# QZ1-boy/FCVSR

Hardware: AMD Instinct MI355X
Metric: SR frames/sec (7-frame window, 4x 180x320->720x1280) + PSNR vs ref (higher is better)
Workload: dtype bf16

## Files before the change

### fcvsr_amd/csrc/conv_mfma.hip

```cpp
#include <stdlib.h>
#include "common.h"
#include "mfma_util.h"
#include "conv_res.h"

namespace fcvsr {

constexpr int kTW = 32, kCK = 64, kLD = kCK + 8;

struct MGroup {
  View src[3];
  View res[2];
  View dst;
  float* gc_partial;
  int B, H, W;
  int tiles_x, tiles_y;
  int tile_begin;
};

struct MfmaArgs {
  int n_groups;
  MGroup g[3];
  int n_src, n_res;
  int seg_c[3];
  int cin_total, cin16, cin_pad, cout, cout_pad, n_nblk;
  const uint16_t* w;
  const float* bias;
  int act;
  float slope;
  const float* slope_ptr;
  float rs[2];
  int ps;
  int flat;
  int src16, dst16;
  int dstbf;
  int res16;
  int gc16;
  const float* gc_wmask;
  int planar;
  int sub2;
  int dbg;
};

struct EpiCtx {
  int act, n_res, ps, flat, H, W, b, dst16, dstbf, sub2, cq4;
  float slope, rs0, rs1;
  long long npix;
  View res0, res1, dst;
};

template <bool BF16>
__device__ __forceinline__ bool epilogue_quad(const EpiCtx& e, float4 v, const float* bias, int cout, int n, int py, int px,
                                              long long pflat, float4* xo) {
  bool pok = e.flat ? (pflat < e.npix) : ((py < e.H) && (px < e.W));
  if (e.sub2) {
    pok = pok && !((py | px) & 1);
    py >>= 1;
    px >>= 1;
  }
  if (!pok || n >= cout) return false;
  const bool full = (n + 3 < cout);
  float x[4] = {v.x, v.y, v.z, v.w};
  if (bias) {
    if (full) {
      const float4 b4 = *reinterpret_cast<const float4*>(bias + n);
      x[0] += b4.x; x[1] += b4.y; x[2] += b4.z; x[3] += b4.w;
    } else {
#pragma unroll
      for (int q = 0; q < 4; ++q) if (n + q < cout) x[q] += bias[n + q];
    }
  }
#pragma unroll
  for (int q = 0; q < 4; ++q) {
    x[q] = x[q] >= 0.f ? x[q] : x[q] * e.slope;
  }
  const int sp_r = e.ps ? n / e.cq4 : 0;
  const int c_r = e.ps ? n - sp_r * e.cq4 : n;
#pragma unroll
  for (int ri = 0; ri < 2; ++ri) {
    if (ri < e.n_res) {
      const View& rv = ri == 0 ? e.res0 : e.res1;
      const float rs = ri == 0 ? e.rs0 : e.rs1;
      const int o = (e.flat ? (int)pflat * (int)rv.sx : (e.b * (int)rv.sb + py * (int)rv.sy + px * (int)rv.sx));
      if (full && rv.sc == 1 && !e.ps) {
        const float4 r4 = *reinterpret_cast<const float4*>(rv.p + o + n);
        x[0] = fmaf(rs, r4.x, x[0]); x[1] = fmaf(rs, r4.y, x[1]); x[2] = fmaf(rs, r4.z, x[2]); x[3] = fmaf(rs, r4.w, x[3]);
      } else {
#pragma unroll
        for (int q = 0; q < 4; ++q) {
          const int ch = e.ps ? 4 * (c_r + q) + sp_r : n + q;
          if (n + q < cout) x[q] = fmaf(rs, rv.p[o + ch * (int)rv.sc], x[q]);
        }
      }
    }
  }
  const View& d = e.dst;
  int o;
  int nn = n;
  if (e.ps) {
    int qy = py, qx = px, qb = e.b;
    if (e.flat) {
      qx = (int)(pflat % e.W);
      qy = (int)((pflat / e.W) % e.H);
      qb = (int)(pflat / ((long long)e.W * e.H));
    }
    const int sp = n / e.cq4;
    nn = n - sp * e.cq4;
    o = qb * (int)d.sb + (2 * qy + (sp >> 1)) * (int)d.sy + (2 * qx + (sp & 1)) * (int)d.sx;
  } else {
    o = (e.flat ? (int)pflat * (int)d.sx : (e.b * (int)d.sb + py * (int)d.sy + px * (int)d.sx));
  }
  if (e.dst16) {
    uint16_t* dp = reinterpret_cast<uint16_t*>(d.p);
    const uint2 pk = e.dstbf ? cvt4<true>(make_float4(x[0], x[1], x[2], x[3])) : cvt4<false>(make_float4(x[0], x[1], x[2], x[3]));
    if (full && d.sc == 1) {
      *reinterpret_cast<uint2*>(dp + o + nn) = pk;
    } else {
      const uint16_t hv[4] = {(uint16_t)(pk.x & 0xffff), (uint16_t)(pk.x >> 16), (uint16_t)(pk.y & 0xffff), (uint16_t)(pk.y >> 16)};
#pragma unroll
      for (int q = 0; q < 4; ++q) if (n + q < cout) dp[o + (nn + q) * (int)d.sc] = hv[q];
    }
  } else if (full && d.sc == 1) {
    *reinterpret_cast<float4*>(d.p + o + nn) = make_float4(x[0], x[1], x[2], x[3]);
  } else {
#pragma unroll
    for (int q = 0; q < 4; ++q) if (n + q < cout) d.p[o + (nn + q) * (int)d.sc] = x[q];
  }
  *xo = make_float4(x[0], n + 1 < cout ? x[1] : 0.f, n + 2 < cout ? x[2] : 0.f, n + 3 < cout ? x[3] : 0.f);
  return true;
}

template <bool BF16>
__device__ __forceinline__ void epilogue_oct(const EpiCtx& e, float4 va, float4 vb, const float* bias, int n, int py, int px,
                                             long long pflat) {
  bool pok = e.flat ? (pflat < e.npix) : ((py < e.H) && (px < e.W));
  if (e.sub2) {
    pok = pok && !((py | px) & 1);
    py >>= 1;
    px >>= 1;
  }
  if (!pok) return;
  float x[8] = {va.x, va.y, va.z, va.w, vb.x, vb.y, vb.z, vb.w};
  if (bias) {
    const float4 b0 = *reinterpret_cast<const float4*>(bias + n), b1 = *reinterpret_cast<const float4*>(bias + n + 4);
    x[0] += b0.x; x[1] += b0.y; x[2] += b0.z; x[3] += b0.w; x[4] += b1.x; x[5] += b1.y; x[6] += b1.z; x[7] += b1.w;
  }
#pragma unroll
  for (int q = 0; q < 8; ++q) {
    x[q] = x[q] >= 0.f ? x[q] : x[q] * e.slope;
  }
#pragma unroll
  for (int ri = 0; ri < 2; ++ri) {
    if (ri < e.n_res) {
      const View& rv = ri == 0 ? e.res0 : e.res1;
      const float rs = ri == 0 ? e.rs0 : e.rs1;
      const int o = (e.flat ? (int)pflat * (int)rv.sx : (e.b * (int)rv.sb + py * (int)rv.sy + px * (int)rv.sx));
      if (rv.sc == 1) {
        const float4 r0 = *reinterpret_cast<const float4*>(rv.p + o + n), r1 = *reinterpret_cast<const float4*>(rv.p + o + n + 4);
        x[0] = fmaf(rs, r0.x, x[0]); x[1] = fmaf(rs, r0.y, x[1]); x[2] = fmaf(rs, r0.z, x[2]); x[3] = fmaf(rs, r0.w, x[3]);
        x[4] = fmaf(rs, r1.x, x[4]); x[5] = fmaf(rs, r1.y, x[5]); x[6] = fmaf(rs, r1.z, x[6]); x[7] = fmaf(rs, r1.w, x[7]);
      } else {
#pragma unroll
        for (int q = 0; q < 8; ++q) x[q] = fmaf(rs, rv.p[o + (n + q) * (int)rv.sc], x[q]);
      }
    }
  }
  const View& d = e.dst;
  const int o = (e.flat ? (int)pflat * (int)d.sx : (e.b * (int)d.sb + py * (int)d.sy + px * (int)d.sx));
  uint2 lo, hi;
  if (e.dstbf) { lo = cvt4<true>(make_float4(x[0], x[1], x[2], x[3])); hi = cvt4<true>(make_float4(x[4], x[5], x[6], x[7])); }
  else { lo = cvt4<false>(make_float4(x[0], x[1], x[2], x[3])); hi = cvt4<false>(make_float4(x[4], x[5], x[6], x[7])); }
  *reinterpret_cast<uint4*>(reinterpret_cast<uint16_t*>(d.p) + o + n) = make_uint4(lo.x, lo.y, hi.x, hi.y);
}

__device__ __forceinline__ long long uniform64(long long v) {
  const unsigned lo = __builtin_amdgcn_readfirstlane((unsigned)v), hi = __builtin_amdgcn_readfirstlane((unsigned)((unsigned long long)v >> 32));
  return (long long)(((unsigned long long)hi << 32) | lo);
}
__device__ __forceinline__ long long sel3(int i, long long a, long long b, long long c) { return i == 0 ? a : (i == 1 ? b : c); }
typedef unsigned __attribute__((ext_vector_type(4))) cm_u32x4_t;
typedef float __attribute__((ext_vector_type(4))) cm_f32x4_t;
typedef __attribute__((address_space(1))) cm_u32x4_t cm_guint4_t;
typedef __attribute__((address_space(1))) cm_f32x4_t cm_gfloat4_t;
__device__ __forceinline__ uint4 gld_u4(long long addr) { const cm_u32x4_t v = *reinterpret_cast<const cm_guint4_t*>((unsigned long long)addr); return make_uint4(v.x, v.y, v.z, v.w); }
__device__ __forceinline__ float4 gld_f4(long long addr) { const cm_f32x4_t v = *reinterpret_cast<const cm_gfloat4_t*>((unsigned long long)addr); return make_float4(v.x, v.y, v.z, v.w); }

template <bool BF16, int NT, int KS, int MW, bool WD>
__global__ __launch_bounds__(256, MW == 1 ? (WD ? (NT == 128 ? 2 : 3) : (NT == 128 ? 3 : 4)) : 2) void conv_mfma_kernel(MfmaArgs a) {
  constexpr bool FLAT = KS == 1;
  constexpr int kTH = 4 * MW;
  constexpr int PAD = KS / 2;
  constexpr int HH = kTH + 2 * PAD, HWD = kTW + 2 * PAD;
  constexpr int NF = NT / 32;
  constexpr int WLOADS = NT * kCK * 2 / 16 / 256;
  extern __shared__ __align__(16) uint16_t lds[];
  uint16_t* A_s = lds;
  uint16_t* B_s = lds + HH * HWD * kLD;

  const int tid = threadIdx.x;
  const int lane = tid & 63, wave = tid >> 6;
  const int r = lane & 31, h = lane >> 5;

  int wid = blockIdx.x;
  {
    const int nwg = gridDim.x, q = nwg >> 3, rr = nwg & 7, xcd = wid & 7, loc = wid >> 3;
    wid = (xcd < rr ? xcd * (q + 1) : rr * (q + 1) + (xcd - rr) * q) + loc;
  }
  const int nb = wid % a.n_nblk;
  const int tflat = wid / a.n_nblk;
  int gi = 0;
  if (a.n_groups > 1 && tflat >= a.g[1].tile_begin) gi = 1;
  if (a.n_groups > 2 && tflat >= a.g[2].tile_begin) gi = 2;
  const MGroup& G = a.g[gi];
  const int tl = tflat - G.tile_begin;
  const int n0 = nb * NT;
  int b, ty0, tx0;
  long long flat0 = 0;
  const long long npix = (long long)G.B * G.H * G.W;
  if (a.flat) {
    flat0 = (long long)tl * (kTH * kTW);
    b = 0; ty0 = 0; tx0 = 0;
  } else {
    const int per_img = G.tiles_x * G.tiles_y;
    b = tl / per_img;
    const int t2 = tl % per_img;
    ty0 = (t2 / G.tiles_x) * kTH;
    tx0 = (t2 % G.tiles_x) * kTW;
  }

  f32x16_t acc[MW][NF];
#pragma unroll
  for (int m = 0; m < MW; ++m)
#pragma unroll
    for (int nf = 0; nf < NF; ++nf)
#pragma unroll
      for (int i = 0; i < 16; ++i) acc[m][nf][i] = 0.f;

  for (int c0 = 0; c0 < a.cin16; c0 += kCK) {
    const int ck = (a.cin16 - c0) < kCK ? (a.cin16 - c0) : kCK;
    __syncthreads();
    if (a.planar) {
      constexpr int NHP = HH * HWD;
      const View sv = G.src[0];
      const int cpad = a.cin16;
      for (int idx = tid; idx < NHP * cpad; idx += 256) {
        const int hp = idx % NHP, c = idx / NHP;
        const int hy = hp / HWD, hx = hp - hy * HWD;
        const int iy = ty0 + hy - PAD, ix = tx0 + hx - PAD;
        float v = 0.f;
        if (c < a.cin_total && iy >= 0 && iy < G.H && ix >= 0 && ix < G.W && !(a.dbg & 1))
          v = sv.p[(long long)b * sv.sb + (long long)iy * sv.sy + (long long)ix * sv.sx + (long long)c * sv.sc];
        const uint2 pk = cvt4<BF16>(make_float4(v, 0.f, 0.f, 0.f));
        A_s[hp * kLD + c] = (uint16_t)(pk.x & 0xffff);
      }
    } else if (!a.src16) {
      constexpr int NHP = HH * HWD;
      constexpr int ITERS = (NHP * 16 + 255) / 256;
      const int q = tid & 15;
      const int c = c0 + q * 4;
      const bool cok = (c < a.cin_total) && !(a.dbg & 1);
      int s_ = 0, cl = c;
      if (cl >= a.seg_c[0]) { cl -= a.seg_c[0]; s_ = 1; if (cl >= a.seg_c[1]) { cl -= a.seg_c[1]; s_ = 2; } }
      const int si = cok ? s_ : 0;
      const long long sp0 = sel3(si, uniform64((long long)G.src[0].p), uniform64((long long)G.src[1].p), uniform64((long long)G.src[2].p));
      const long long ssb = sel3(si, uniform64(G.src[0].sb), uniform64(G.src[1].sb), uniform64(G.src[2].sb));
      const long long ssy = sel3(si, uniform64(G.src[0].sy), uniform64(G.src[1].sy), uniform64(G.src[2].sy));
      const long long ssx = sel3(si, uniform64(G.src[0].sx), uniform64(G.src[1].sx), uniform64(G.src[2].sx));
      const long long sbase = sp0 + 4 * ((FLAT ? 0ll : (long long)b * ssb) + (cok ? cl : 0));
      constexpr int UNR = 8;
#pragma unroll 1
      for (int it0 = 0; it0 < ITERS; it0 += UNR) {
        float4 v[UNR];
        bool ok[UNR];
#pragma unroll
        for (int u = 0; u < UNR; ++u) {
          const int hp = (tid >> 4) + (it0 + u) * 16;
          long long off;
          if (FLAT) {
            const long long p = flat0 + hp;
            ok[u] = cok && hp < NHP && p < npix;
            off = (p < npix ? p : npix - 1) * ssx;
          } else {
            const int hy = hp / HWD, hx = hp - hy * HWD;
            const int iy = ty0 + hy - PAD, ix = tx0 + hx - PAD;
            ok[u] = cok && hp < NHP && iy >= 0 && iy < G.H && ix >= 0 && ix < G.W;
            const int cy = iy < 0 ? 0 : (iy > G.H - 1 ? G.H - 1 : iy), cx = ix < 0 ? 0 : (ix > G.W - 1 ? G.W - 1 : ix);
            off = (long long)cy * ssy + (long long)cx * ssx;
          }
          v[u] = gld_f4(sbase + 4 * off);
        }
#pragma unroll
        for (int u = 0; u < UNR; ++u)
          if (!ok[u]) v[u] = make_float4(0.f, 0.f, 0.f, 0.f);
#pragma unroll
        for (int u = 0; u < UNR; ++u) {
          const int hp = (tid >> 4) + (it0 + u) * 16;
          if (hp < NHP) *reinterpret_cast<uint2*>(A_s + hp * kLD + q * 4) = cvt4<BF16>(v[u]);
        }
      }
    } else {
      constexpr int NHP = HH * HWD;
      constexpr int ITERS = (NHP * 8 + 255) / 256;
      const int q = tid & 7;
      const int c = c0 + q * 8;
      const bool cok = (c < a.cin_total) && !(a.dbg & 1);
      int s_ = 0, cl = c;
      if (cl >= a.seg_c[0]) { cl -= a.seg_c[0]; s_ = 1; if (cl >= a.seg_c[1]) { cl -= a.seg_c[1]; s_ = 2; } }
      const int si = cok ? s_ : 0;
      const long long sp0 = sel3(si, uniform64((long long)G.src[0].p), uniform64((long long)G.src[1].p), uniform64((long long)G.src[2].p));
      const long long ssb = sel3(si, uniform64(G.src[0].sb), uniform64(G.src[1].sb), uniform64(G.src[2].sb));
      const long long ssy = sel3(si, uniform64(G.src[0].sy), uniform64(G.src[1].sy), uniform64(G.src[2].sy));
      const long long ssx = sel3(si, uniform64(G.src[0].sx), uniform64(G.src[1].sx), uniform64(G.src[2].sx));
      const long long sbase = sp0 + 2 * ((FLAT ? 0ll : (long long)b * ssb) + (cok ? cl : 0));
      constexpr int UNR = 8;
#pragma unroll 1
      for (int it0 = 0; it0 < ITERS; it0 += UNR) {
        uint4 v[UNR];
        bool ok[UNR];
#pragma unroll
        for (int u = 0; u < UNR; ++u) {
          const int hp = (tid >> 3) + (it0 + u) * 32;
          long long off;
          if (FLAT) {
            const long long p = flat0 + hp;
            ok[u] = cok && hp < NHP && p < npix;
            off = (p < npix ? p : npix - 1) * ssx;
          } else {
            const int hy = hp / HWD, hx = hp - hy * HWD;
            const int iy = ty0 + hy - PAD, ix = tx0 + hx - PAD;
            ok[u] = cok && hp < NHP && iy >= 0 && iy < G.H && ix >= 0 && ix < G.W;
            const int cy = iy < 0 ? 0 : (iy > G.H - 1 ? G.H - 1 : iy), cx = ix < 0 ? 0 : (ix > G.W - 1 ? G.W - 1 : ix);
            off = (long long)cy * ssy + (long long)cx * ssx;
          }
          v[u] = gld_u4(sbase + 2 * off);
        }
#pragma unroll
        for (int u = 0; u < UNR; ++u)
          if (!ok[u]) v[u] = make_uint4(0, 0, 0, 0);
#pragma unroll
        for (int u = 0; u < UNR; ++u) {
          const int hp = (tid >> 3) + (it0 + u) * 32;
          if (hp < NHP) *reinterpret_cast<uint4*>(A_s + hp * kLD + q * 8) = v[u];
        }
      }
    }
    if (WD) {
      constexpr int S = KS * KS * 4;
      constexpr int PD = NT == 128 ? 3 : 4;
      const long long wtap = (long long)a.cout_pad * a.cin_pad;
      const long long wrow32 = 32ll * a.cin_pad;
      const uint16_t* wl = a.w + ((long long)n0 + r) * a.cin_pad + c0 + h * 8;
      uint4 bq[PD][NF];
#pragma unroll
      for (int s0 = 0; s0 < PD && s0 < S; ++s0) {
        const int tap = s0 >> 2, kk = s0 & 3;
        if (kk * 16 < ck && !(a.dbg & 8)) {
#pragma unroll
          for (int nf = 0; nf < NF; ++nf)
            bq[s0][nf] = *reinterpret_cast<const uint4*>(wl + tap * wtap + nf * wrow32 + kk * 16);
        }
      }
      __syncthreads();
#pragma unroll
      for (int s1 = 0; s1 < S; ++s1) {
        const int tap = s1 >> 2, kk = s1 & 3;
        const int ky = tap / KS, kx = tap - ky * KS;
        if (kk * 16 < ck && !(a.dbg & 2)) {
          const uint16_t* arow0 = A_s + ((MW * wave + ky) * HWD + r + kx) * kLD + h * 8;
          uint4 af[MW];
#pragma unroll
          for (int m = 0; m < MW; ++m) af[m] = *reinterpret_cast<const uint4*>(arow0 + m * HWD * kLD + kk * 16);
#pragma unroll
          for (int m = 0; m < MW; ++m)
#pragma unroll
            for (int nf = 0; nf < NF; ++nf) acc[m][nf] = mfma<BF16>(af[m], bq[s1 % PD][nf], acc[m][nf]);
        }
        if (s1 + PD < S) {
          const int tap2 = (s1 + PD) >> 2, kk2 = (s1 + PD) & 3;
          if (kk2 * 16 < ck && !(a.dbg & 8)) {
#pragma unroll
            for (int nf = 0; nf < NF; ++nf)
              bq[s1 % PD][nf] = *reinterpret_cast<const uint4*>(wl + tap2 * wtap + nf * wrow32 + kk2 * 16);
          }
        }
      }
    } else {
    uint4 w0 = make_uint4(0, 0, 0, 0), w1 = w0, w2 = w0, w3 = w0;
    const uint16_t* wbase = a.w + ((long long)n0 + (tid >> 3)) * a.cin_pad + c0 + (tid & 7) * 8;
    const long long wtap = (long long)a.cout_pad * a.cin_pad;
    const long long wrow32 = 32ll * a.cin_pad;
#define FCVSR_FETCH_W(TAP)                                                                             \
  do {                                                                                                 \
    const uint16_t* wp_ = wbase + (TAP) * wtap;                                                        \
    if (a.dbg & 8) break;                                                                              \
    w0 = *reinterpret_cast<const uint4*>(wp_);                                                         \
    if (WLOADS > 1) w1 = *reinterpret_cast<const uint4*>(wp_ + wrow32);                                \
    if (WLOADS > 2) w2 = *reinterpret_cast<const uint4*>(wp_ + 2 * wrow32);                            \
    if (WLOADS > 3) w3 = *reinterpret_cast<const uint4*>(wp_ + 3 * wrow32);                            \
  } while (0)
    FCVSR_FETCH_W(0);
#pragma unroll 1
    for (int tap = 0; tap < KS * KS; ++tap) {
      if (tap > 0) __syncthreads();
      {
        uint16_t* bp = B_s + (tid >> 3) * kLD + (tid & 7) * 8;
        *reinterpret_cast<uint4*>(bp) = w0;
        if (WLOADS > 1) *reinterpret_cast<uint4*>(bp + 32 * kLD) = w1;
        if (WLOADS > 2) *reinterpret_cast<uint4*>(bp + 64 * kLD) = w2;
        if (WLOADS > 3) *reinterpret_cast<uint4*>(bp + 96 * kLD) = w3;
      }
      __syncthreads();
      if (tap + 1 < KS * KS) FCVSR_FETCH_W(tap + 1);
      const int ky = tap / KS, kx = tap - ky * KS;
      const uint16_t* arow0 = A_s + ((MW * wave + ky) * HWD + r + kx) * kLD + h * 8;
      const uint16_t* brow = B_s + r * kLD + h * 8;
#pragma unroll
      for (int kk = 0; kk < kCK / 16; ++kk) {
        if (kk * 16 < ck && !(a.dbg & 2)) {
          uint4 af[MW], bf[NF];
#pragma unroll
          for (int m = 0; m < MW; ++m) af[m] = *reinterpret_cast<const uint4*>(arow0 + m * HWD * kLD + kk * 16);
#pragma unroll
          for (int nf = 0; nf < NF; ++nf) bf[nf] = *reinterpret_cast<const uint4*>(brow + nf * 32 * kLD + kk * 16);
#pragma unroll
          for (int m = 0; m < MW; ++m)
#pragma unroll
            for (int nf = 0; nf < NF; ++nf) acc[m][nf] = mfma<BF16>(af[m], bf[nf], acc[m][nf]);
        }
      }
    }
    }
  }

  float slope = a.slope;
  if (a.act == FCVSR_ACT_PRELU) slope = *reinterpret_cast<const __attribute__((address_space(1))) float*>(reinterpret_cast<uintptr_t>(a.slope_ptr));
  EpiCtx e;
  e.act = a.act; e.slope = a.act == FCVSR_ACT_RELU ? 0.f : (a.act == FCVSR_ACT_NONE ? 1.f : slope); e.n_res = a.n_res; e.rs0 = a.rs[0]; e.rs1 = a.rs[1]; e.ps = a.ps; e.flat = a.flat;
  e.res0 = G.res[0]; e.res1 = G.res[1]; e.dst = G.dst; e.H = G.H; e.W = G.W; e.b = b; e.npix = npix;
  e.dst16 = a.dst16; e.dstbf = a.dstbf; e.cq4 = a.cout >> 2; e.sub2 = a.sub2;
  constexpr int EW = NT >= 64 ? 64 : 32;
  constexpr int EROW = EW + 4;
  constexpr int QPR = EW / 4;
  __syncthreads();
  float* E_s = reinterpret_cast<float*>(lds) + wave * (32 * EROW);
  const bool oct_path = a.dst16 && !a.ps && !a.gc_wmask && (a.cout % 8 == 0) && G.dst.sc == 1;
#pragma unroll
  for (int m = 0; m < MW; ++m) {
    const int yo = MW * wave + m;
#pragma unroll
    for (int nh = 0; nh < NT / EW; ++nh) {
#pragma unroll
      for (int nf2 = 0; nf2 < EW / 32; ++nf2) {
#pragma unroll
        for (int i = 0; i < 16; ++i)
          E_s[((i & 3) + 8 * (i >> 2) + 4 * h) * EROW + nf2 * 32 + r] = acc[m][nh * (EW / 32) + nf2][i];
      }
      __builtin_amdgcn_wave_barrier();
      float gm = -INFINITY, gs = 0.f;
      float4 ga = make_float4(0.f, 0.f, 0.f, 0.f);
      if (oct_path) {
        constexpr int OPR = EW / 8;
#pragma unroll
        for (int j = 0; j < 32 * OPR / 64; ++j) {
          const int idx = j * 64 + lane;
          const int co = idx % OPR, p = idx / OPR;
          const float4 va = *reinterpret_cast<const float4*>(E_s + p * EROW + co * 8);
          const float4 vb = *reinterpret_cast<const float4*>(E_s + p * EROW + co * 8 + 4);
          const int n = n0 + nh * EW + co * 8;
          if (n < a.cout && (!(a.dbg & 4) || va.x == 12345.678f))
            epilogue_oct<BF16>(e, va, vb, a.bias, n, ty0 + yo, tx0 + p, flat0 + yo * kTW + p);
          asm volatile("" ::: "memory");
        }
      } else
#pragma unroll
      for (int j = 0; j < 32 * QPR / 64; ++j) {
        const int idx = j * 64 + lane;
        const int cq = idx % QPR, p = idx / QPR;
        const float4 v = *reinterpret_cast<const float4*>(E_s + p * EROW + cq * 4);
        const int n = n0 + nh * EW + cq * 4;
        float4 xo = make_float4(0.f, 0.f, 0.f, 0.f);
        bool valid = false;
        if (!(a.dbg & 4) || v.x == 12345.678f)
          valid = epilogue_quad<BF16>(e, v, a.bias, a.cout, n, ty0 + yo, tx0 + p, flat0 + yo * kTW + p, &xo);
        if (a.gc_wmask) {
          float part = 0.f;
          if (valid) {
            const float4 wm = *reinterpret_cast<const float4*>(a.gc_wmask + n);
            part = xo.x * wm.x + (n + 1 < a.cout ? xo.y * wm.y : 0.f) + (n + 2 < a.cout ? xo.z * wm.z : 0.f) +
                   (n + 3 < a.cout ? xo.w * wm.w : 0.f);
          }
#pragma unroll
          for (int o = QPR / 2; o >= 1; o >>= 1) part += __shfl_xor(part, o);
          const bool pval = (ty0 + yo < G.H) && (tx0 + p < G.W);
          if (pval) {
            const float mn = fmaxf(gm, part);
            const float sc = expf(gm - mn);
            const float ee = expf(part - mn);
            gs = gs * sc + ee;
            ga.x = ga.x * sc + ee * xo.x; ga.y = ga.y * sc + ee * xo.y; ga.z = ga.z * sc + ee * xo.z; ga.w = ga.w * sc + ee * xo.w;
            gm = mn;
          }
        }
        asm volatile("" ::: "memory");
      }
      if (a.gc_wmask && G.gc_partial) {
#pragma unroll
        for (int o = QPR; o < 64; o <<= 1) {
          const float om = __shfl_xor(gm, o), os = __shfl_xor(gs, o);
          const float ox = __shfl_xor(ga.x, o), oy = __shfl_xor(ga.y, o), oz = __shfl_xor(ga.z, o), ow = __shfl_xor(ga.w, o);
          const float mn = fmaxf(gm, om);
          const float s1 = (gm == -INFINITY) ? 0.f : expf(gm - mn), s2 = (om == -INFINITY) ? 0.f : expf(om - mn);
          gs = gs * s1 + os * s2;
          ga.x = ga.x * s1 + ox * s2; ga.y = ga.y * s1 + oy * s2; ga.z = ga.z * s1 + oz * s2; ga.w = ga.w * s1 + ow * s2;
          gm = mn;
        }
        float* gw = reinterpret_cast<float*>(lds) + 4 * 32 * EROW + wave * (EW + 4);
        if (lane < QPR) {
          *reinterpret_cast<float4*>(gw + lane * 4) = ga;
          if (lane == 0) { gw[EW] = gm; gw[EW + 1] = gs; }
        }
      }
      __builtin_amdgcn_wave_barrier();
    }
  }
  if (a.gc_wmask && G.gc_partial && NT <= 64 && MW == 1) {
    __syncthreads();
    if (wave == 0 && lane < QPR) {
      const float* g0 = reinterpret_cast<const float*>(lds) + 4 * 32 * EROW;
      float m = -INFINITY;
#pragma unroll
      for (int w = 0; w < 4; ++w) m = fmaxf(m, g0[w * (EW + 4) + EW]);
      float sum = 0.f;
      float4 acc4 = make_float4(0.f, 0.f, 0.f, 0.f);
#pragma unroll
      for (int w = 0; w < 4; ++w) {
        const float mw = g0[w * (EW + 4) + EW];
        const float sc = (mw == -INFINITY) ? 0.f : expf(mw - m);
        sum = fmaf(g0[w * (EW + 4) + EW + 1], sc, sum);
        const float4 v = *reinterpret_cast<const float4*>(g0 + w * (EW + 4) + lane * 4);
        acc4.x = fmaf(v.x, sc, acc4.x); acc4.y = fmaf(v.y, sc, acc4.y); acc4.z = fmaf(v.z, sc, acc4.z); acc4.w = fmaf(v.w, sc, acc4.w);
      }
      const int per_img = G.tiles_x * G.tiles_y;
      float* pp = G.gc_partial + ((long long)b * per_img + (tl % per_img)) * (a.cout + 2);
      const int n = lane * 4;
      if (n < a.cout) pp[n] = acc4.x;
      if (n + 1 < a.cout) pp[n + 1] = acc4.y;
      if (n + 2 < a.cout) pp[n + 2] = acc4.z;
      if (n + 3 < a.cout) pp[n + 3] = acc4.w;
      if (lane == 0) { pp[a.cout] = m; pp[a.cout + 1] = sum; }
    }
  }
}

template <bool BF16, int NT, bool SRC16, bool DST16>
__global__ __launch_bounds__(256, NT == 128 ? 2 : 4) void conv3_lean_kernel(MfmaArgs a) {
  constexpr int HWD = kTW + 2, NHP = 6 * HWD;
  constexpr int NF = NT / 32;
  constexpr int WLOADS = NT / 32;
  extern __shared__ __align__(16) uint16_t lds[];
  uint16_t* A_s = lds;
  uint16_t* B_s = lds + NHP * kLD;
  const int tid = threadIdx.x;
  const int lane = tid & 63, wave = tid >> 6;
  const int r = lane & 31, h = lane >> 5;

  int wid = blockIdx.x;
  {
    const int nwg = gridDim.x, q = nwg >> 3, rr = nwg & 7, xcd = wid & 7, loc = wid >> 3;
    wid = (xcd < rr ? xcd * (q + 1) : rr * (q + 1) + (xcd - rr) * q) + loc;
  }
  const int nb = wid % a.n_nblk;
  const int tflat = wid / a.n_nblk;
  int gi = 0;
  if (a.n_groups > 1 && tflat >= a.g[1].tile_begin) gi = 1;
  if (a.n_groups > 2 && tflat >= a.g[2].tile_begin) gi = 2;
  const MGroup& G = a.g[gi];
  const int tl = tflat - G.tile_begin;
  const int n0 = nb * NT;
  const int per_img = G.tiles_x * G.tiles_y;
  const int b = tl / per_img;
  const int t2 = tl - b * per_img;
  const int ty0 = (t2 / G.tiles_x) * 4, tx0 = (t2 % G.tiles_x) * kTW;
  const int H = G.H, W = G.W;

  f32x16_t acc[NF];
#pragma unroll
  for (int nf = 0; nf < NF; ++nf)
#pragma unroll
    for (int i = 0; i < 16; ++i) acc[nf][i] = 0.f;

  constexpr int EPL = SRC16 ? 8 : 4;
  constexpr int LPP = 64 / EPL;
  constexpr int STEP = 256 / LPP;
  constexpr int ITERS = (NHP + STEP - 1) / STEP;
  const int q = tid & (LPP - 1);
  const int p0 = tid / LPP;
  const View sv = G.src[0];
  const int ssx = (int)sv.sx, ssy = (int)sv.sy;
  constexpr int ESZ = SRC16 ? 2 : 4;
  const char* sbase = reinterpret_cast<const char*>(sv.p) + ((long long)b * sv.sb) * ESZ;
  const int off0 = ((ty0 - 1) * ssy + (tx0 - 1 + p0) * ssx + q * EPL) * ESZ;
  uint16_t* a_dst = A_s + p0 * kLD + q * EPL;

  for (int c0 = 0; c0 < a.cin16; c0 += kCK) {
    const int ck = (a.cin16 - c0) < kCK ? (a.cin16 - c0) : kCK;
    __syncthreads();
    {
      int hy = 0, hx = p0, off = off0 + c0 * ESZ;
      const bool cok = (c0 + q * EPL) < a.cin_total;
      constexpr int SB = 7;
#pragma unroll
      for (int i0 = 0; i0 < ITERS; i0 += SB) {
        uint4 v[SB];
#pragma unroll
        for (int u = 0; u < SB; ++u) {
          const int i = i0 + u;
          v[u] = make_uint4(0, 0, 0, 0);
          if (i < ITERS) {
            const int iy = ty0 + hy - 1, ix = tx0 + hx - 1;
            const bool ok = cok && (p0 + i * STEP < NHP) && ((unsigned)iy < (unsigned)H) && ((unsigned)ix < (unsigned)W);
            const uint4 ld = *reinterpret_cast<const uint4*>(sbase + (ok ? (unsigned)off : 0u));
            if (ok) v[u] = ld;
            hx += STEP;
            off += STEP * ssx * ESZ;
            if (hx >= HWD) { hx -= HWD; ++hy; off += (ssy - HWD * ssx) * ESZ; }
          }
        }
#pragma unroll
        for (int u = 0; u < SB; ++u) {
          const int i = i0 + u;
          if (i < ITERS && p0 + i * STEP < NHP) {
            if (SRC16) {
              *reinterpret_cast<uint4*>(a_dst + i * STEP * kLD) = v[u];
            } else {
              const float4 f = __builtin_bit_cast(float4, v[u]);
              *reinterpret_cast<uint2*>(a_dst + i * STEP * kLD) = cvt4<BF16>(f);
            }
          }
        }
      }
    }
    uint4 w0 = make_uint4(0, 0, 0, 0), w1 = w0, w2 = w0, w3 = w0;
    const uint16_t* wbase = a.w + ((long long)n0 + (tid >> 3)) * a.cin_pad + c0 + (tid & 7) * 8;
    const long long wtap = (long long)a.cout_pad * a.cin_pad;
    const long long wrow32 = 32ll * a.cin_pad;
#define FCVSR_FETCH_WL(TAP)                                                       \
  do {                                                                            \
    const uint16_t* wp_ = wbase + (TAP) * wtap;                                   \
    w0 = *reinterpret_cast<const uint4*>(wp_);                                    \
    if (WLOADS > 1) w1 = *reinterpret_cast<const uint4*>(wp_ + wrow32);           \
    if (WLOADS > 2) w2 = *reinterpret_cast<const uint4*>(wp_ + 2 * wrow32);       \
    if (WLOADS > 3) w3 = *reinterpret_cast<const uint4*>(wp_ + 3 * wrow32);       \
  } while (0)
    FCVSR_FETCH_WL(0);
    uint16_t* bp = B_s + (tid >> 3) * kLD + (tid & 7) * 8;
    const uint16_t* arow = A_s + (wave * HWD + r) * kLD + h * 8;
    const uint16_t* brow = B_s + r * kLD + h * 8;
#pragma unroll
    for (int tap = 0; tap < 9; ++tap) {
      if (tap > 0) __syncthreads();
      *reinterpret_cast<uint4*>(bp) = w0;
      if (WLOADS > 1) *reinterpret_cast<uint4*>(bp + 32 * kLD) = w1;
      if (WLOADS > 2) *reinterpret_cast<uint4*>(bp + 64 * kLD) = w2;
      if (WLOADS > 3) *reinterpret_cast<uint4*>(bp + 96 * kLD) = w3;
      __syncthreads();
      if (tap + 1 < 9) FCVSR_FETCH_WL(tap + 1);
      const int ky = tap / 3, kx = tap % 3;
#pragma unroll
      for (int kk = 0; kk < kCK / 16; ++kk) {
        if (kk * 16 < ck) {
          const uint4 af = *reinterpret_cast<const uint4*>(arow + (ky * HWD + kx) * kLD + kk * 16);
          uint4 bf[NF];
#pragma unroll
          for (int nf = 0; nf < NF; ++nf) bf[nf] = *reinterpret_cast<const uint4*>(brow + nf * 32 * kLD + kk * 16);
#pragma unroll
          for (int nf = 0; nf < NF; ++nf) acc[nf] = mfma<BF16>(af, bf[nf], acc[nf]);
        }
      }
    }
  }

  float slope = a.slope;
  if (a.act == FCVSR_ACT_PRELU) slope = *reinterpret_cast<const __attribute__((address_space(1))) float*>(reinterpret_cast<uintptr_t>(a.slope_ptr));
  const int act = a.act;
  const float nsf = act == FCVSR_ACT_RELU ? 0.f : (act == FCVSR_ACT_NONE ? 1.f : slope);
  constexpr int EW = NT >= 64 ? 64 : 32;
  constexpr int EROW = EW + 4;
  __syncthreads();
  float* E_s = reinterpret_cast<float*>(lds) + wave * (32 * EROW);
  const int py = ty0 + wave;
  const bool rowok = py < H;
  const View dv = G.dst;
  const View r0v = G.res[0], r1v = G.res[1];
  const int dsx = (int)dv.sx, r0sx = (int)r0v.sx, r1sx = (int)r1v.sx;
  const long long drow = (long long)b * dv.sb + (long long)py * dv.sy;
  const long long r0off = (long long)b * r0v.sb + (long long)py * r0v.sy;
  const long long r1off = (long long)b * r1v.sb + (long long)py * r1v.sy;
  const bool r16 = a.res16 != 0;
  float gm = -INFINITY, gs = 0.f;
  float4 ga = make_float4(0.f, 0.f, 0.f, 0.f);
#pragma unroll
  for (int nh = 0; nh < NT / EW; ++nh) {
#pragma unroll
    for (int nf2 = 0; nf2 < EW / 32; ++nf2) {
#pragma unroll
      for (int i = 0; i < 16; ++i)
        E_s[((i & 3) + 8 * (i >> 2) + 4 * h) * EROW + nf2 * 32 + r] = acc[nh * (EW / 32) + nf2][i];
    }
    __builtin_amdgcn_wave_barrier();
    if (DST16) {
      constexpr int OPR = EW / 8;
      const int co = lane & (OPR - 1), psub = lane / OPR;
      const int n = n0 + nh * EW + co * 8;
      const bool nok = n < a.cout;
      float4 b0 = make_float4(0.f, 0.f, 0.f, 0.f), b1 = b0;
      if (a.bias && nok) { b0 = *reinterpret_cast<const float4*>(a.bias + n); b1 = *reinterpret_cast<const float4*>(a.bias + n + 4); }
      uint16_t* dp = reinterpret_cast<uint16_t*>(dv.p) + drow + n;
      const float* es = E_s + psub * EROW + co * 8;
      constexpr int PPI = 64 / OPR;
#pragma unroll
      for (int j = 0; j < 32 / PPI; ++j) {
        const int px = tx0 + j * PPI + psub;
        if (rowok && nok && px < W) {
          const float4 va = *reinterpret_cast<const float4*>(es + j * PPI * EROW);
          const float4 vb = *reinterpret_cast<const float4*>(es + j * PPI * EROW + 4);
          float x[8] = {va.x + b0.x, va.y + b0.y, va.z + b0.z, va.w + b0.w, vb.x + b1.x, vb.y + b1.y, vb.z + b1.z, vb.w + b1.w};
#pragma unroll
          for (int k = 0; k < 8; ++k) x[k] = x[k] >= 0.f ? x[k] : x[k] * nsf;
          if (a.n_res > 0) {
            float rr[8];
            load_res<BF16, 8>(r0v.p, r0off + px * r0sx + n, r16, rr);
#pragma unroll
            for (int k = 0; k < 8; ++k) x[k] = fmaf(a.rs[0], rr[k], x[k]);
          }
          if (a.n_res > 1) {
            float rr[8];
            load_res<BF16, 8>(r1v.p, r1off + px * r1sx + n, r16, rr);
#pragma unroll
            for (int k = 0; k < 8; ++k) x[k] = fmaf(a.rs[1], rr[k], x[k]);
          }
          const uint2 lo = cvt4<BF16>(make_float4(x[0], x[1], x[2], x[3])), hi = cvt4<BF16>(make_float4(x[4], x[5], x[6], x[7]));
          *reinterpret_cast<uint4*>(dp + px * dsx) = make_uint4(lo.x, lo.y, hi.x, hi.y);
        }
      }
    } else {
      constexpr int QPR = EW / 4;
      const int cq = lane & (QPR - 1), psub = lane / QPR;
      const int n = n0 + nh * EW + cq * 4;
      const bool nok = n < a.cout;
      const bool full = n + 3 < a.cout;
      const bool vec = full && dv.sc == 1 && (a.n_res < 1 || r0v.sc == 1) && (a.n_res < 2 || r1v.sc == 1);
      float4 b0 = make_float4(0.f, 0.f, 0.f, 0.f);
      if (a.bias && nok) {
        if (full) b0 = *reinterpret_cast<const float4*>(a.bias + n);
        else { b0.x = a.bias[n]; if (n + 1 < a.cout) b0.y = a.bias[n + 1]; if (n + 2 < a.cout) b0.z = a.bias[n + 2]; }
      }
      float4 wm = make_float4(0.f, 0.f, 0.f, 0.f);
      if (a.gc_wmask && nok) wm = *reinterpret_cast<const float4*>(a.gc_wmask + n);
      float* dp = dv.p + drow + n;
      const float* es = E_s + psub * EROW + cq * 4;
      constexpr int PPI = 64 / QPR;
#pragma unroll
      for (int j = 0; j < 32 / PPI; ++j) {
        const int px = tx0 + j * PPI + psub;
        const bool pval = rowok && px < W;
        float4 x = make_float4(0.f, 0.f, 0.f, 0.f);
        if (pval && nok) {
          const float4 va = *reinterpret_cast<const float4*>(es + j * PPI * EROW);
          x = make_float4(va.x + b0.x, va.y + b0.y, va.z + b0.z, va.w + b0.w);
          x.x = x.x >= 0.f ? x.x : x.x * nsf; x.y = x.y >= 0.f ? x.y : x.y * nsf;
          x.z = x.z >= 0.f ? x.z : x.z * nsf; x.w = x.w >= 0.f ? x.w : x.w * nsf;
          if (vec) {
            if (a.n_res > 0) {
              float rr[4];
              load_res<BF16, 4>(r0v.p, r0off + px * r0sx + n, r16, rr);
              x.x = fmaf(a.rs[0], rr[0], x.x); x.y = fmaf(a.rs[0], rr[1], x.y); x.z = fmaf(a.rs[0], rr[2], x.z); x.w = fmaf(a.rs[0], rr[3], x.w);
            }
            if (a.n_res > 1) {
              float rr[4];
              load_res<BF16, 4>(r1v.p, r1off + px * r1sx + n, r16, rr);
              x.x = fmaf(a.rs[1], rr[0], x.x); x.y = fmaf(a.rs[1], rr[1], x.y); x.z = fmaf(a.rs[1], rr[2], x.z); x.w = fmaf(a.rs[1], rr[3], x.w);
            }
            if (a.gc16) *reinterpret_cast<uint2*>(reinterpret_cast<uint16_t*>(dv.p) + drow + n + px * dsx) = cvt4<BF16>(x);
            else *reinterpret_cast<float4*>(dp + px * dsx) = x;
          } else {
            float xs[4] = {x.x, x.y, x.z, x.w};
#pragma unroll
            for (int k = 0; k < 4; ++k) {
              if (n + k < a.cout) {
                if (a.n_res > 0) xs[k] = fmaf(a.rs[0], r0v.p[r0off + px * r0sx + (long long)(n + k) * r0v.sc], xs[k]);
                if (a.n_res > 1) xs[k] = fmaf(a.rs[1], r1v.p[r1off + px * r1sx + (long long)(n + k) * r1v.sc], xs[k]);
                dv.p[drow + px * dsx + (long long)(n + k) * dv.sc] = xs[k];
              } else {
                xs[k] = 0.f;
              }
            }
            x = make_float4(xs[0], xs[1], xs[2], xs[3]);
          }
        }
        if (a.gc_wmask) {
          float part = x.x * wm.x + x.y * wm.y + x.z * wm.z + x.w * wm.w;
#pragma unroll
          for (int o = QPR / 2; o >= 1; o >>= 1) part += __shfl_xor(part, o);
          if (pval) {
            const float mn = fmaxf(gm, part);
            const float sc = expf(gm - mn), ee = expf(part - mn);
            gs = gs * sc + ee;
            ga.x = ga.x * sc + ee * x.x; ga.y = ga.y * sc + ee * x.y; ga.z = ga.z * sc + ee * x.z; ga.w = ga.w * sc + ee * x.w;
            gm = mn;
          }
        }
      }
      if (a.gc_wmask && G.gc_partial) {
#pragma unroll
        for (int o = QPR; o < 64; o <<= 1) {
          const float om = __shfl_xor(gm, o), os = __shfl_xor(gs, o);
          const float ox = __shfl_xor(ga.x, o), oy = __shfl_xor(ga.y, o), oz = __shfl_xor(ga.z, o), ow = __shfl_xor(ga.w, o);
          const float mn = fmaxf(gm, om);
          const float s1 = (gm == -INFINITY) ? 0.f : expf(gm - mn), s2 = (om == -INFINITY) ? 0.f : expf(om - mn);
          gs = gs * s1 + os * s2;
          ga.x = ga.x * s1 + ox * s2; ga.y = ga.y * s1 + oy * s2; ga.z = ga.z * s1 + oz * s2; ga.w = ga.w * s1 + ow * s2;
          gm = mn;
        }
        float* gw = reinterpret_cast<float*>(lds) + 4 * 32 * EROW + wave * (EW + 4);
        if (lane < QPR) {
          *reinterpret_cast<float4*>(gw + lane * 4) = ga;
          if (lane == 0) { gw[EW] = gm; gw[EW + 1] = gs; }
        }
      }
    }
    __builtin_amdgcn_wave_barrier();
  }
  if (!DST16 && a.gc_wmask && G.gc_partial && NT <= 64) {
    constexpr int QPR = EW / 4;
    __syncthreads();
    if (wave == 0 && lane < QPR) {
      const float* g0 = reinterpret_cast<const float*>(lds) + 4 * 32 * EROW;
      float m = -INFINITY;
#pragma unroll
      for (int w = 0; w < 4; ++w) m = fmaxf(m, g0[w * (EW + 4) + EW]);
      float sum = 0.f;
      float4 acc4 = make_float4(0.f, 0.f, 0.f, 0.f);
#pragma unroll
      for (int w = 0; w < 4; ++w) {
        const float mw = g0[w * (EW + 4) + EW];
        const float sc = (mw == -INFINITY) ? 0.f : expf(mw - m);
        sum = fmaf(g0[w * (EW + 4) + EW + 1], sc, sum);
        const float4 v = *reinterpret_cast<const float4*>(g0 + w * (EW + 4) + lane * 4);
        acc4.x = fmaf(v.x, sc, acc4.x); acc4.y = fmaf(v.y, sc, acc4.y); acc4.z = fmaf(v.z, sc, acc4.z); acc4.w = fmaf(v.w, sc, acc4.w);
      }
      float* pp = G.gc_partial + ((long long)b * per_img + t2) * (a.cout + 2);
      const int n = lane * 4;
      if (n < a.cout) pp[n] = acc4.x;
      if (n + 1 < a.cout) pp[n + 1] = acc4.y;
      if (n + 2 < a.cout) pp[n + 2] = acc4.z;
      if (n + 3 < a.cout) pp[n + 3] = acc4.w;
      if (lane == 0) { pp[a.cout] = m; pp[a.cout + 1] = sum; }
    }
  }
}

template <bool BF16, int NT, bool SRC16, bool DST16, bool PS>
__global__ __launch_bounds__(256, 4) void conv1_lean_kernel(MfmaArgs a) {
  constexpr int NPX = 128;
  constexpr int NF = NT / 32;
  constexpr int WLOADS = NT / 32;
  extern __shared__ __align__(16) uint16_t lds[];
  uint16_t* A_s = lds;
  uint16_t* B_s = lds + NPX * kLD;
  const int tid = threadIdx.x;
  const int lane = tid & 63, wave = tid >> 6;
  const int r = lane & 31, h = lane >> 5;
  int wid = blockIdx.x;
  {
    const int nwg = gridDim.x, q = nwg >> 3, rr = nwg & 7, xcd = wid & 7, loc = wid >> 3;
    wid = (xcd < rr ? xcd * (q + 1) : rr * (q + 1) + (xcd - rr) * q) + loc;
  }
  const int nb = wid % a.n_nblk;
  const int tflat = wid / a.n_nblk;
  int gi = 0;
  if (a.n_groups > 1 && tflat >= a.g[1].tile_begin) gi = 1;
  if (a.n_groups > 2 && tflat >= a.g[2].tile_begin) gi = 2;
  const MGroup& G = a.g[gi];
  const int tl = tflat - G.tile_begin;
  const int n0 = nb * NT;
  const int npix = G.B * G.H * G.W;
  const int flat0 = tl * NPX;

  f32x16_t acc[NF];
#pragma unroll
  for (int nf = 0; nf < NF; ++nf)
#pragma unroll
    for (int i = 0; i < 16; ++i) acc[nf][i] = 0.f;

  constexpr int EPL = SRC16 ? 8 : 4;
  constexpr int LPP = 64 / EPL;
  constexpr int STEP = 256 / LPP;
  constexpr int ITERS = NPX / STEP;
  constexpr int ESZ = SRC16 ? 2 : 4;
  const int q = tid & (LPP - 1);
  const int p0 = tid / LPP;
  uint16_t* a_dst = A_s + p0 * kLD + q * EPL;

  for (int c0 = 0; c0 < a.cin16; c0 += kCK) {
    int sidx = 0, cl = c0;
    if (cl >= a.seg_c[0]) { cl -= a.seg_c[0]; sidx = 1; if (cl >= a.seg_c[1]) { cl -= a.seg_c[1]; sidx = 2; } }
    const View sv = G.src[sidx];
    const char* sbase = reinterpret_cast<const char*>(sv.p) + (cl + q * EPL) * ESZ;
    const int ssx = (int)sv.sx;
    __syncthreads();
    {
      uint4 v[ITERS];
#pragma unroll
      for (int i = 0; i < ITERS; ++i) {
        const int pix = flat0 + p0 + i * STEP;
        const long long pc = pix < npix ? pix : npix - 1;
        v[i] = *reinterpret_cast<const uint4*>(sbase + (size_t)((unsigned)pc * (unsigned)ssx) * ESZ);
      }
#pragma unroll
      for (int i = 0; i < ITERS; ++i) {
        if (SRC16) {
          *reinterpret_cast<uint4*>(a_dst + i * STEP * kLD) = v[i];
        } else {
          *reinterpret_cast<uint2*>(a_dst + i * STEP * kLD) = cvt4<BF16>(__builtin_bit_cast(float4, v[i]));
        }
      }
    }
    {
      const uint16_t* wp_ = a.w + ((long long)n0 + (tid >> 3)) * a.cin_pad + c0 + (tid & 7) * 8;
      const long long wrow32 = 32ll * a.cin_pad;
      uint16_t* bp = B_s + (tid >> 3) * kLD + (tid & 7) * 8;
      const uint4 w0 = *reinterpret_cast<const uint4*>(wp_);
      uint4 w1 = w0;
      if (WLOADS > 1) w1 = *reinterpret_cast<const uint4*>(wp_ + wrow32);
      *reinterpret_cast<uint4*>(bp) = w0;
      if (WLOADS > 1) *reinterpret_cast<uint4*>(bp + 32 * kLD) = w1;
    }
    __syncthreads();
    const uint16_t* arow = A_s + (wave * 32 + r) * kLD + h * 8;
    const uint16_t* brow = B_s + r * kLD + h * 8;
#pragma unroll
    for (int kk = 0; kk < kCK / 16; ++kk) {
      const uint4 af = *reinterpret_cast<const uint4*>(arow + kk * 16);
      uint4 bf[NF];
#pragma unroll
      for (int nf = 0; nf < NF; ++nf) bf[nf] = *reinterpret_cast<const uint4*>(brow + nf * 32 * kLD + kk * 16);
#pragma unroll
      for (int nf = 0; nf < NF; ++nf) acc[nf] = mfma<BF16>(af, bf[nf], acc[nf]);
    }
  }

  float slope = a.slope;
  if (a.act == FCVSR_ACT_PRELU) slope = *reinterpret_cast<const __attribute__((address_space(1))) float*>(reinterpret_cast<uintptr_t>(a.slope_ptr));
  const int act = a.act;
  const float nsf = act == FCVSR_ACT_RELU ? 0.f : (act == FCVSR_ACT_NONE ? 1.f : slope);
  constexpr int EW = NT >= 64 ? 64 : 32;
  constexpr int EROW = EW + 4;
  __syncthreads();
  float* E_s = reinterpret_cast<float*>(lds) + wave * (32 * EROW);
  const int rowpix = flat0 + wave * 32;
  const View dv = G.dst;
  const View r0v = G.res[0], r1v = G.res[1];
  const int dsx = (int)dv.sx, r0sx = (int)r0v.sx, r1sx = (int)r1v.sx;
  const int cq4 = a.cout >> 2;
#pragma unroll
  for (int nf2 = 0; nf2 < EW / 32; ++nf2) {
#pragma unroll
    for (int i = 0; i < 16; ++i) E_s[((i & 3) + 8 * (i >> 2) + 4 * h) * EROW + nf2 * 32 + r] = acc[nf2][i];
  }
  __builtin_amdgcn_wave_barrier();
  constexpr int VPL = DST16 ? 8 : 4;
  constexpr int LPR = EW / VPL;
  constexpr int PPI = 64 / LPR;
  const int co = lane & (LPR - 1), psub = lane / LPR;
  const int n = n0 + co * VPL;
  const bool nok = n < a.cout;
  float bb[VPL];
#pragma unroll
  for (int k = 0; k < VPL; ++k) bb[k] = 0.f;
  if (a.bias && nok) {
#pragma unroll
    for (int k = 0; k < VPL; k += 4) {
      const float4 t = *reinterpret_cast<const float4*>(a.bias + n + k);
      bb[k] = t.x; bb[k + 1] = t.y; bb[k + 2] = t.z; bb[k + 3] = t.w;
    }
  }
  const int sp = PS ? n / cq4 : 0;
  const int nn = PS ? n - sp * cq4 : n;
  const float* es = E_s + psub * EROW + co * VPL;
#pragma unroll
  for (int j = 0; j < 32 / PPI; ++j) {
    const int pix = rowpix + j * PPI + psub;
    if (nok && pix < npix) {
      float x[VPL];
#pragma unroll
      for (int k = 0; k < VPL; k += 4) {
        const float4 t = *reinterpret_cast<const float4*>(es + j * PPI * EROW + k);
        x[k] = t.x + bb[k]; x[k + 1] = t.y + bb[k + 1]; x[k + 2] = t.z + bb[k + 2]; x[k + 3] = t.w + bb[k + 3];
      }
#pragma unroll
      for (int k = 0; k < VPL; ++k) x[k] = x[k] >= 0.f ? x[k] : x[k] * nsf;
      if (!PS) {
        if (a.n_res > 0) {
#pragma unroll
          for (int k = 0; k < VPL; k += 4) {
            const float4 t = *reinterpret_cast<const float4*>(r0v.p + (size_t)((unsigned)pix * (unsigned)r0sx) + n + k);
            x[k] = fmaf(a.rs[0], t.x, x[k]); x[k + 1] = fmaf(a.rs[0], t.y, x[k + 1]);
            x[k + 2] = fmaf(a.rs[0], t.z, x[k + 2]); x[k + 3] = fmaf(a.rs[0], t.w, x[k + 3]);
          }
        }
        if (a.n_res > 1) {
#pragma unroll
          for (int k = 0; k < VPL; k += 4) {
            const float4 t = *reinterpret_cast<const float4*>(r1v.p + (size_t)((unsigned)pix * (unsigned)r1sx) + n + k);
            x[k] = fmaf(a.rs[1], t.x, x[k]); x[k + 1] = fmaf(a.rs[1], t.y, x[k + 1]);
            x[k + 2] = fmaf(a.rs[1], t.z, x[k + 2]); x[k + 3] = fmaf(a.rs[1], t.w, x[k + 3]);
          }
        }
      }
      size_t o;
      if (PS) {
        const int qx = pix % G.W, t1 = pix / G.W;
        const int qy = t1 % G.H, qb = t1 / G.H;
        o = (size_t)qb * dv.sb + (size_t)(2 * qy + (sp >> 1)) * dv.sy + (size_t)(2 * qx + (sp & 1)) * dsx + nn;
      } else {
        o = (size_t)((unsigned)pix * (unsigned)dsx) + n;
      }
      if (DST16) {
        const uint2 lo = cvt4<BF16>(make_float4(x[0], x[1], x[2], x[3]));
        const uint2 hi = cvt4<BF16>(make_float4(x[VPL - 4], x[VPL - 3], x[VPL - 2], x[VPL - 1]));
        *reinterpret_cast<uint4*>(reinterpret_cast<uint16_t*>(dv.p) + o) = make_uint4(lo.x, lo.y, hi.x, hi.y);
      } else {
        *reinterpret_cast<float4*>(dv.p + o) = make_float4(x[0], x[1], x[2], x[3]);
      }
    }
  }
}

template <bool BF16, int NT, bool SRC16, bool DST16, bool PS>
static hipError_t launch_lean1(const MfmaArgs& a, int total_tiles, hipStream_t st) {
  size_t lds = ((size_t)128 * kLD + (size_t)NT * kLD) * sizeof(uint16_t);
  const size_t epi = 4ull * 32 * ((NT >= 64 ? 64 : 32) + 4) * sizeof(float);
  if (lds < epi) lds = epi;
  hipLaunchKernelGGL((conv1_lean_kernel<BF16, NT, SRC16, DST16, PS>), dim3(total_tiles * a.n_nblk), dim3(256), lds, st, a);
  return hipGetLastError();
}

template <bool BF16>
static hipError_t dispatch_lean1(const MfmaArgs& a, int nt, int total_tiles, hipStream_t st) {
#define FCVSR_L1(NTV, PSV)                                                                                      \
  (a.src16 ? (a.dst16 ? launch_lean1<BF16, NTV, true, true, PSV>(a, total_tiles, st)                              \
                      : launch_lean1<BF16, NTV, true, false, PSV>(a, total_tiles, st))                            \
           : (a.dst16 ? launch_lean1<BF16, NTV, false, true, PSV>(a, total_tiles, st)                             \
                      : launch_lean1<BF16, NTV, false, false, PSV>(a, total_tiles, st)))
  if (a.ps) return nt == 64 ? FCVSR_L1(64, true) : FCVSR_L1(32, true);
  return nt == 64 ? FCVSR_L1(64, false) : FCVSR_L1(32, false);
#undef FCVSR_L1
}

template <bool BF16, int NT, bool SRC16, bool DST16>
static hipError_t launch_lean(const MfmaArgs& a, int total_tiles, hipStream_t st) {
  size_t lds = ((size_t)6 * (kTW + 2) * kLD + (size_t)NT * kLD) * sizeof(uint16_t);
  const size_t epi = (4ull * 32 + 4) * ((NT >= 64 ? 64 : 32) + 4) * sizeof(float);
  if (lds < epi) lds = epi;
  static DevOnce attr;
  hipError_t e = once_per_device(attr, [&] {
    return hipFuncSetAttribute((const void*)conv3_lean_kernel<BF16, NT, SRC16, DST16>, hipFuncAttributeMaxDynamicSharedMemorySize, (int)lds);
  });
  if (e != hipSuccess) return e;
  hipLaunchKernelGGL((conv3_lean_kernel<BF16, NT, SRC16, DST16>), dim3(total_tiles * a.n_nblk), dim3(256), lds, st, a);
  return hipGetLastError();
}

template <bool BF16>
static hipError_t dispatch_lean(const MfmaArgs& a, int nt, int total_tiles, hipStream_t st) {
#define FCVSR_LEAN(NTV)                                                                                       \
  (a.src16 ? (a.dst16 ? launch_lean<BF16, NTV, true, true>(a, total_tiles, st)                                  \
                      : launch_lean<BF16, NTV, true, false>(a, total_tiles, st))                                \
           : (a.dst16 ? launch_lean<BF16, NTV, false, true>(a, total_tiles, st)                                 \
                      : launch_lean<BF16, NTV, false, false>(a, total_tiles, st)))
  if (nt == 64) return FCVSR_LEAN(64);
  return FCVSR_LEAN(32);
#undef FCVSR_LEAN
}

template <bool BF16, int NT, int KS, int MW, bool WD>
static hipError_t launch_mfma(const MfmaArgs& a, int total_tiles, hipStream_t st) {
  constexpr int PAD = KS / 2;
  constexpr int kTH = 4 * MW;
  size_t lds = ((size_t)(kTH + 2 * PAD) * (kTW + 2 * PAD) * kLD + (size_t)NT * kLD) * sizeof(uint16_t);
  const size_t epi = (4ull * 32 + 4) * ((NT >= 64 ? 64 : 32) + 4) * sizeof(float);
  if (lds < epi) lds = epi;
  static DevOnce attr;
  hipError_t e = once_per_device(attr, [&] {
    return hipFuncSetAttribute((const void*)conv_mfma_kernel<BF16, NT, KS, MW, WD>, hipFuncAttributeMaxDynamicSharedMemorySize, (int)lds);
  });
  if (e != hipSuccess) return e;
  hipLaunchKernelGGL((conv_mfma_kernel<BF16, NT, KS, MW, WD>), dim3(total_tiles * a.n_nblk), dim3(256), lds, st, a);
  return hipGetLastError();
}

template <bool BF16, int MW, bool WD>
static hipError_t dispatch2(const MfmaArgs& a, int nt, int ks, int total_tiles, hipStream_t st) {
  if (ks == 3) {
    if (nt == 64) return launch_mfma<BF16, 64, 3, MW, WD>(a, total_tiles, st);
    return launch_mfma<BF16, 32, 3, MW, WD>(a, total_tiles, st);
  }
  if (nt == 64) return launch_mfma<BF16, 64, 1, MW, WD>(a, total_tiles, st);
  return launch_mfma<BF16, 32, 1, MW, WD>(a, total_tiles, st);
}

template <bool BF16>
static hipError_t dispatch(const MfmaArgs& a, int nt, int ks, int mw, int wd, int total_tiles, hipStream_t st) {
  (void)mw;
  return wd ? dispatch2<BF16, 1, true>(a, nt, ks, total_tiles, st) : dispatch2<BF16, 1, false>(a, nt, ks, total_tiles, st);
}

}

using namespace fcvsr;

static void* g_res_stamps = nullptr;
static const size_t kResStampBytes = 8 * 64 * 8 * sizeof(unsigned long long);
extern "C" int fcvsr_debug_res_stamps(void* host_out, size_t bytes) {
  if (!g_res_stamps || bytes > kResStampBytes) return FCVSR_E_ARG;
  return (int)hipMemcpy(host_out, g_res_stamps, bytes, hipMemcpyDeviceToHost);
}

static thread_local char g_last_kernel[96] = "";
extern "C" const char* fcvsr_last_conv_kernel(void) { return g_last_kernel; }
#define FCVSR_NOTE_KERNEL(...) snprintf(g_last_kernel, sizeof(g_last_kernel), __VA_ARGS__)
static const char* tf(int v) { return v ? "true" : "false"; }

static bool vec_view_ok(const fcvsr_view& v) {
  const int g = v.dtype == FCVSR_F32 ? 4 : 8;
  return v.sc != 1 || v.c < 4 || (v.sx % 4 == 0 && v.sy % 4 == 0 && v.sb % 4 == 0 && ((uintptr_t)v.ptr % (g == 4 ? 16 : 8)) == 0);
}

static bool src_ok(const fcvsr_view& v, int mma_dtype) {
  if (!v.ptr || v.sc != 1 || ((uintptr_t)v.ptr % 16) != 0) return false;
  const int g = v.dtype == FCVSR_F32 ? 4 : 8;
  if (v.dtype != FCVSR_F32 && v.dtype != mma_dtype) return false;
  return v.c % g == 0 && v.sx % g == 0 && v.sy % g == 0 && v.sb % g == 0;
}

extern "C" int fcvsr_conv2d_mfma(const fcvsr_conv_desc* descs, int n_groups, int mma_dtype, void* stream) {
  FCVSR_CHECK_ARG(descs != nullptr && n_groups >= 1 && n_groups <= 3, "1..3 problem groups");
  FCVSR_CHECK_ARG(mma_dtype == FCVSR_BF16 || mma_dtype == FCVSR_F16, "mma_dtype must be BF16 or F16");
  const fcvsr_conv_desc& d0 = descs[0];
  FCVSR_CHECK_ARG(d0.kh == d0.kw && (d0.kh == 1 || d0.kh == 3) && d0.pad == d0.kh / 2 &&
                      (d0.stride == 1 || (d0.stride == 2 && d0.kh == 3 && !d0.pixel_shuffle)),
                  "MFMA path: 1x1 or 3x3 stride 1, or 3x3 stride 2, same padding");
  FCVSR_CHECK_ARG(d0.n_src >= 1 && d0.n_src <= 3 && d0.n_res >= 0 && d0.n_res <= 2 && d0.cout > 0, "bad descriptor");
  FCVSR_CHECK_ARG(d0.weight != nullptr && d0.cout_pad % 128 == 0 && d0.cout_pad >= d0.cout, "weight must be MFMA-packed");
  FCVSR_CHECK_ARG(!(d0.act == FCVSR_ACT_PRELU) || d0.slope_ptr != nullptr, "PReLU needs slope_ptr");
  FCVSR_CHECK_ARG(!d0.pixel_shuffle || d0.cout % 16 == 0, "pixel_shuffle needs cout%16==0 (sub-pixel-major packing)");
  MfmaArgs a;
  a.src16 = d0.src[0].dtype != FCVSR_F32;
  a.res16 = (d0.n_res > 0 && d0.res[0].dtype != FCVSR_F32) ? 1 : 0;
  a.sub2 = d0.stride == 2;
  a.planar = (d0.n_src == 1 && d0.src[0].sc != 1) ? 1 : 0;
  FCVSR_CHECK_ARG(!a.planar || (d0.src[0].dtype == FCVSR_F32 && d0.src[0].c <= 32 && d0.kh == 3),
                  "planar (channel-strided) source: one f32 source with <= 32 channels, 3x3");
  a.dst16 = d0.dst.dtype != FCVSR_F32;
  a.gc16 = 0;
  a.dstbf = d0.dst.dtype == FCVSR_BF16;
  const bool dst_native = d0.dst.dtype == FCVSR_F32 || d0.dst.dtype == mma_dtype;
  a.n_groups = n_groups;
  a.n_src = d0.n_src;
  a.n_res = d0.n_res;
  int cin = 0;
  for (int s = 0; s < 3; ++s) {
    a.seg_c[s] = s < d0.n_src ? d0.src[s].c : (1 << 30);
    if (s < d0.n_src) cin += d0.src[s].c;
  }
  a.cin_total = cin;
  a.cin16 = (cin + 15) / 16 * 16;
  a.cin_pad = (cin + 63) / 64 * 64;
  a.cout = d0.cout;
  a.cout_pad = d0.cout_pad;
  int nt = d0.cout > 32 ? 64 : 32;
  a.n_nblk = (d0.cout + nt - 1) / nt;
  a.w = (const uint16_t*)d0.weight;
  a.bias = d0.bias;
  a.act = d0.act;
  a.slope = d0.slope;
  a.slope_ptr = d0.slope_ptr;
  a.rs[0] = d0.res_scale[0];
  a.rs[1] = d0.res_scale[1];
  a.ps = d0.pixel_shuffle;
  a.flat = d0.kh == 1 ? 1 : 0;
  a.gc_wmask = d0.gc_wmask;
  FCVSR_CHECK_ARG(d0.gc_wmask == nullptr || (d0.kh == 3 && d0.stride == 1 && d0.cout <= 64 && !d0.pixel_shuffle &&
                                             ((uintptr_t)d0.gc_wmask % 16) == 0),
                  "ContextBlock fusion: 3x3 stride-1 layer with cout <= 64");
  {
    const char* dbg = getenv("FCVSR_MFMA_DBG");
    a.dbg = dbg ? atoi(dbg) : 0;
  }
  const int mw = 1;
  int wd = 0;
  {
    const char* e = getenv("FCVSR_MFMA_WD");
    if (e) wd = atoi(e) ? 1 : 0;
  }
  const int kTH = 4 * mw;
  int tiles = 0;
  for (int g = 0; g < n_groups; ++g) {
    const fcvsr_conv_desc& d = descs[g];
    FCVSR_CHECK_ARG(d.kh == d0.kh && d.kw == d0.kw && d.stride == d0.stride && d.n_src == d0.n_src && d.n_res == d0.n_res &&
                        d.cout == d0.cout && d.weight == d0.weight && d.bias == d0.bias && d.act == d0.act &&
                        d.pixel_shuffle == d0.pixel_shuffle,
                    "groups must share weights and epilogue");
    FCVSR_CHECK_ARG(d.B > 0 && d.H > 0 && d.W > 0, "empty problem");
    MGroup& G = a.g[g];
    for (int s = 0; s < d.n_src; ++s) {
      FCVSR_CHECK_ARG((a.planar ? (d.src[s].ptr != nullptr && d.src[s].sc != 1) : src_ok(d.src[s], mma_dtype)) &&
                          d.src[s].c == d0.src[s].c && d.src[s].dtype == d0.src[0].dtype,
                      "src: f32 or MFMA dtype (all alike), channel-contiguous, 16-byte aligned, c%4==0 (f32) / c%8==0 (16-bit)");
      G.src[s] = to_view(d.src[s]);
      if (a.flat)
        FCVSR_CHECK_ARG(d.src[s].sy == d.src[s].sx * d.W && d.src[s].sb == d.src[s].sy * d.H, "1x1 needs uniformly strided pixels");
    }
    for (int q = 0; q < d.n_res; ++q) {
      FCVSR_CHECK_ARG(d.res[q].ptr && (d.res[q].dtype == FCVSR_F32 || d.res[q].dtype == mma_dtype) &&
                          d.res[q].dtype == d0.res[0].dtype && vec_view_ok(d.res[q]),
                      "res must be f32 or the MFMA dtype (all alike), vector-aligned");
      G.res[q] = to_view(d.res[q]);
      if (a.flat)
        FCVSR_CHECK_ARG(d.res[q].sy == d.res[q].sx * d.W && d.res[q].sb == d.res[q].sy * d.H, "1x1 needs uniformly strided res");
    }
    FCVSR_CHECK_ARG(d.dst.ptr && (d.dst.dtype == FCVSR_F32 || d.dst.dtype == FCVSR_BF16 || d.dst.dtype == FCVSR_F16) &&
                        d.dst.dtype == d0.dst.dtype && vec_view_ok(d.dst), "dst must be f32 / bf16 / f16, vector-aligned");
    FCVSR_CHECK_ARG(d.bias == nullptr || ((uintptr_t)d.bias % 16) == 0, "bias must be 16-byte aligned");
    G.dst = to_view(d.dst);
    if (a.flat && !d.pixel_shuffle)
      FCVSR_CHECK_ARG(d.dst.sy == d.dst.sx * d.W && d.dst.sb == d.dst.sy * d.H, "1x1 needs uniformly strided dst");
    G.gc_partial = d.gc_partial;
    FCVSR_CHECK_ARG((d.gc_wmask == nullptr) == (d.gc_partial == nullptr) && d.gc_wmask == d0.gc_wmask, "gc fields: all groups alike");
    G.B = d.B; G.H = d.H; G.W = d.W;
    G.tile_begin = tiles;
    if (a.flat) {
      G.tiles_x = 1; G.tiles_y = 1;
      tiles += cdiv((long long)d.B * d.H * d.W, kTH * kTW);
    } else {
      G.tiles_x = cdiv(d.W, kTW);
      G.tiles_y = cdiv(d.H, kTH);
      tiles += d.B * G.tiles_x * G.tiles_y;
    }
  }
  for (int g = n_groups; g < 3; ++g) a.g[g] = a.g[0];
  hipStream_t st = (hipStream_t)stream;
  bool lean = dst_native && d0.kh == 3 && d0.stride == 1 && mw == 1 && !wd && d0.n_src == 1 && !a.planar && !a.ps && (cin % 64 == 0) &&
              (!a.dst16 || d0.cout % 8 == 0) && (d0.gc_wmask == nullptr || d0.cout % 4 == 0);
  for (int g = 0; g < n_groups && lean; ++g) {
    const fcvsr_conv_desc& d = descs[g];
    long long ext = (long long)d.B * d.H * d.W * (long long)(d.src[0].sx > d.dst.sx ? d.src[0].sx : d.dst.sx);
    if (d.dst.sc != 1) ext = (long long)d.B * d.dst.sb;
    lean = lean && (!a.dst16 || d.dst.sc == 1) && ext < (1ll << 29);
    for (int q = 0; q < d.n_res; ++q)
      lean = lean && (d.res[q].dtype == FCVSR_F32 || d.res[q].sc == 1) && (!a.dst16 || d.res[q].sc == 1);
  }
  if (d0.gc_wmask != nullptr && a.dst16) {
    bool ok16 = lean && dst_native && d0.n_res == 0 && d0.cout % 4 == 0;
    for (int g = 0; g < n_groups; ++g) ok16 = ok16 && descs[g].dst.sc == 1;
    FCVSR_CHECK_ARG(ok16, "ContextBlock fusion with a 16-bit destination needs the lean 3x3 path, no residuals");
    a.gc16 = 1;
    a.dst16 = 0;
  }
  FCVSR_CHECK_ARG(!a.res16 || lean, "16-bit residuals are only supported by the lean 3x3 path");
  {
    const char* e = getenv("FCVSR_MFMA_LEAN");
    if (e && atoi(e) == 0) lean = false;
  }
  bool lean1 = dst_native && d0.kh == 1 && mw == 1 && !wd && nt <= 64 && (d0.cout % 8 == 0) && !a.planar;
  for (int s2 = 0; s2 < d0.n_src && lean1; ++s2) lean1 = lean1 && (d0.src[s2].c % 64 == 0);
  lean1 = lean1 && (!a.ps || (d0.n_res == 0 && (d0.cout / 4) % 8 == 0));
  for (int g = 0; g < n_groups && lean1; ++g) {
    const fcvsr_conv_desc& d = descs[g];
    long long maxsx = d.dst.sx;
    for (int s2 = 0; s2 < d.n_src; ++s2) maxsx = d.src[s2].sx > maxsx ? d.src[s2].sx : maxsx;
    lean1 = lean1 && d.dst.sc == 1 && (long long)d.B * d.H * d.W * maxsx * 4 < (1ll << 31);
    for (int q = 0; q < d.n_res; ++q)
      lean1 = lean1 && d.res[q].sc == 1 && d.res[q].dtype == FCVSR_F32 && (long long)d.B * d.H * d.W * d.res[q].sx < (1ll << 31);
  }
  {
    const char* e2 = getenv("FCVSR_MFMA_LEAN");
    if (e2 && atoi(e2) == 0) lean1 = false;
  }
  hipError_t e;
  if (lean1) {
    FCVSR_NOTE_KERNEL("conv1_lean_kernel<%s, %d, %s, %s, %s>", tf(mma_dtype == FCVSR_BF16), nt, tf(a.src16), tf(a.dst16), tf(a.ps));
    e = (mma_dtype == FCVSR_BF16) ? dispatch_lean1<true>(a, nt, tiles, st) : dispatch_lean1<false>(a, nt, tiles, st);
    if (e != hipSuccess) {
      set_error("fcvsr_conv2d_mfma: launch failed: %s", hipGetErrorString(e));
      return (int)e;
    }
    return 0;
  }
  const bool res_ps = a.ps && dst_native && d0.kh == 3 && d0.stride == 1 && mw == 1 && !wd && d0.n_src == 1 && !a.planar && cin == 64 &&
                      d0.cout % 256 == 0 && d0.n_res == 0 && a.dst16 && a.src16 && d0.gc_wmask == nullptr;
  bool res = (lean || res_ps) && a.src16 && conv3_res_supports(cin, d0.cout) && d0.gc_wmask == nullptr && d0.cout == d0.cout / 64 * 64;
  int rtiles = 0;
  for (int g = 0; g < n_groups && res; ++g) {
    const fcvsr_conv_desc& d = descs[g];
    const int dg = a.dst16 ? 8 : 4;
    res = res && d.dst.sc == 1 && d.dst.sx % dg == 0 && d.dst.sy % dg == 0 && d.dst.sb % dg == 0 && ((uintptr_t)d.dst.ptr % 16) == 0;
    res = res && d.src[0].sx % 8 == 0 && d.src[0].sy % 8 == 0 && d.src[0].sb % 8 == 0;
    for (int q = 0; q < d.n_res; ++q) {
      const int rg = d.res[q].dtype == FCVSR_F32 ? 4 : 8;
      res = res && d.res[q].sc == 1 && d.res[q].sx % rg == 0 && d.res[q].sy % rg == 0 && d.res[q].sb % rg == 0 &&
            ((uintptr_t)d.res[q].ptr % 16) == 0;
    }
    rtiles += conv3_res_tiles(d.B, d.H, d.W);
    if (res_ps) res = res && d.dst.c == d0.cout / 4 && (long long)d.B * d.dst.sb < (1ll << 30) && (long long)d.B * d.src[0].sb < (1ll << 29) &&
                      d.src[0].sc == 1 && ((uintptr_t)d.src[0].ptr % 16) == 0;
  }
  {
    const char* e3 = getenv("FCVSR_MFMA_RES");
    const int res_mode = e3 ? (atoi(e3) ? 1 : 0) : 2;
    const char* e4 = getenv("FCVSR_MFMA_RES_MIN");
    const int res_min = e4 ? atoi(e4) : 768;
    if (res_mode == 0 || (res_mode == 2 && rtiles * (cin == 64 ? d0.cout / 64 : d0.cout / 32) < res_min)) res = false;
  }
  if (res) {
    static void* zeros_dev[64] = {nullptr};
    int dev = 0;
    if (hipGetDevice(&dev) != hipSuccess || dev < 0 || dev >= 64) { set_error("fcvsr_conv2d_mfma: bad device index"); return FCVSR_E_ARG; }
    if (!zeros_dev[dev]) {
      hipStreamCaptureStatus cs = hipStreamCaptureStatusNone;
      if (hipStreamIsCapturing(st, &cs) == hipSuccess && cs != hipStreamCaptureStatusNone) {
        set_error("fcvsr_conv2d_mfma: first use on this device inside a stream capture (run the layer once eagerly first)");
        return FCVSR_E_ARG;
      }
      void* z = nullptr;
      hipError_t ez = hipMalloc(&z, 256);
      if (ez == hipSuccess) ez = hipMemset(z, 0, 256);
      if (ez != hipSuccess) {
        set_error("fcvsr_conv2d_mfma: zero page allocation failed: %s", hipGetErrorString(ez));
        return (int)ez;
      }
      zeros_dev[dev] = z;
    }
    void* zeros = zeros_dev[dev];
    ResArgs wa;
    wa.n_groups = n_groups;
    int wtiles = 0;
    for (int g = 0; g < 3; ++g) {
      const MGroup& G = a.g[g < n_groups ? g : 0];
      ResGroup& Wg = wa.g[g];
      Wg.src = G.src[0]; Wg.res[0] = G.res[0]; Wg.res[1] = G.res[1]; Wg.dst = G.dst; Wg.gc_partial = nullptr;
      Wg.B = G.B; Wg.H = G.H; Wg.W = G.W;
      Wg.tiles_x = cdiv(G.W, 32);
      Wg.tiles_y = cdiv(G.H, 8);
      Wg.tile_begin = wtiles;
      if (g < n_groups) wtiles += G.B * Wg.tiles_x * Wg.tiles_y;
    }
    wa.total_tiles = wtiles;
    wa.cin = cin; wa.cout = d0.cout; wa.cout_pad = d0.cout_pad; wa.cin_pad = a.cin_pad;
    wa.w = a.w; wa.bias = a.bias; wa.act = a.act; wa.slope = a.slope; wa.slope_ptr = a.slope_ptr;
    wa.rs[0] = a.rs[0]; wa.rs[1] = a.rs[1]; wa.n_res = a.n_res; wa.res16 = a.res16; wa.ps = a.ps; wa.zeros = zeros;
    { const char* wd_ = getenv("FCVSR_RES_DBG"); wa.dbg = wd_ ? atoi(wd_) : 0; }
    { const char* wv_ = getenv("FCVSR_RES_V"); wa.variant = wv_ ? atoi(wv_) : 1; }
    wa.stamps = nullptr;
    {
      const char* ws_ = getenv("FCVSR_RES_STAMPS");
      if (ws_ && atoi(ws_)) {
        if (!g_res_stamps && hipMalloc(&g_res_stamps, kResStampBytes) != hipSuccess) g_res_stamps = nullptr;
        if (g_res_stamps) (void)hipMemsetAsync(g_res_stamps, 0, kResStampBytes, st);
        wa.stamps = (unsigned long long*)g_res_stamps;
      }
    }
    FCVSR_NOTE_KERNEL((wa.variant >= 3 && mma_dtype == FCVSR_BF16 && a.dst16 && a.n_res == 0) ? "conv3_res3_kernel<%s, %d, %d, %d>" : "conv3_res_kernel<%s, %d, %d, %d>", tf(mma_dtype == FCVSR_BF16), !a.dst16 ? 0 : (a.n_res == 0 ? 2 : 1), cin / 64,
                      a.act == FCVSR_ACT_NONE ? 2 : ((a.act == FCVSR_ACT_RELU || (a.act == FCVSR_ACT_LEAKY && a.slope >= 0.f && a.slope <= 1.f)) ? 1 : 0));
    e = launch_conv3_res(wa, mma_dtype == FCVSR_BF16, a.dst16 != 0, st);
    if (e != hipSuccess) {
      set_error("fcvsr_conv2d_mfma: resident-weight launch failed: %s", hipGetErrorString(e));
      return (int)e;
    }
    return 0;
  }
  if (lean && nt > 64) {
    nt = 64;
    a.n_nblk = (d0.cout + nt - 1) / nt;
  }
  if (lean) FCVSR_NOTE_KERNEL("conv3_lean_kernel<%s, %d, %s, %s>%s", tf(mma_dtype == FCVSR_BF16), nt, tf(a.src16), tf(a.dst16), a.gc_wmask ? " +gc" : "");
  else FCVSR_NOTE_KERNEL("conv_mfma_kernel<%s, %d, %d, %d, %s>", tf(mma_dtype == FCVSR_BF16), nt, d0.kh, mw, tf(wd));
  if (lean) e = (mma_dtype == FCVSR_BF16) ? dispatch_lean<true>(a, nt, tiles, st) : dispatch_lean<false>(a, nt, tiles, st);
  else e = (mma_dtype == FCVSR_BF16) ? dispatch<true>(a, nt, d0.kh, mw, wd, tiles, st) : dispatch<false>(a, nt, d0.kh, mw, wd, tiles, st);
  if (e != hipSuccess) {
    set_error("fcvsr_conv2d_mfma: launch failed: %s", hipGetErrorString(e));
    return (int)e;
  }
  return 0;
}
```

### fcvsr_amd/csrc/conv_res.h

```cpp
#pragma once
#include "common.h"

namespace fcvsr {

struct ResGroup {
  View src, res[2], dst;
  float* gc_partial;
  int B, H, W;
  int tiles_x, tiles_y;
  int tile_begin;
};

struct ResArgs {
  int n_groups;
  ResGroup g[3];
  int total_tiles;
  int cin, cout, cout_pad, cin_pad;
  const uint16_t* w;
  const float* bias;
  int act;
  float slope;
  const float* slope_ptr;
  float rs[2];
  int n_res, res16;
  int ps;
  const void* zeros;
  int variant;
  int dbg;
  unsigned long long* stamps;
};

hipError_t launch_conv3_res(const ResArgs& a, bool bf16, bool dst16, hipStream_t st);
bool conv3_res_supports(int cin, int cout);
inline int conv3_res_tiles(int B, int H, int W) { return B * ((H + 7) / 8) * ((W + 31) / 32); }

}
```

### fcvsr_amd/csrc/conv_res.hip

```cpp
#include <stdlib.h>
#include <type_traits>
#include "conv_res.h"
#include "mfma_util.h"

namespace fcvsr {

constexpr int kRTH = 8, kRTW = 32, kRHW = kRTW + 2, kRHH = kRTH + 2;
constexpr int kRNHP = kRHH * kRHW;
constexpr int kRNG = (kRNHP + 7) / 8;
constexpr int kRXBytes = kRNG * 1024;
constexpr int kRWRows = 576;
constexpr int kRWBytes = kRWRows * 128;
constexpr int kRRowB = kRHW * 128;
constexpr int kRBiasOff = kRWBytes + 2 * kRXBytes;
constexpr int kRTabOff = kRBiasOff + 256;
constexpr size_t kRLds = (size_t)kRTabOff + 3 * 32 * 4;

enum {
  kTSrcLo = 0, kTSrcHi, kTSrcSb2, kTSrcSy2, kTSrcSx2, kTH, kTW, kTTilesX, kTPerImg, kTTileBegin,
  kTDstLo = 12, kTDstHi, kTDstSb, kTDstSy, kTDstSx, kTR0Lo, kTR0Hi, kTR0Sb, kTR0Sy, kTR0Sx, kTR1Lo, kTR1Hi, kTR1Sb, kTR1Sy, kTR1Sx
};

struct ResK {
  int n_groups, total_tiles, cout, cout_pad, cin_pad, act, n_res, res16, dbg, ps;
  float slope, rs[2];
  const float* slope_ptr;
  const uint16_t* w;
  const float* bias;
  const void* zeros;
  unsigned long long* stamps;
  int tab[3][32];
};

struct ResTile {
  int gi, b, ty0, tx0;
};

__device__ __forceinline__ ResTile res_decode(const int* tabL, int n_groups, int tile) {
  ResTile t;
  t.gi = 0;
  if (n_groups > 1 && tile >= tabL[32 + kTTileBegin]) t.gi = 1;
  if (n_groups > 2 && tile >= tabL[64 + kTTileBegin]) t.gi = 2;
  const int* T = tabL + t.gi * 32;
  const int tl = tile - T[kTTileBegin];
  const int per_img = T[kTPerImg], tiles_x = T[kTTilesX];
  t.b = tl / per_img;
  const int t2 = tl - t.b * per_img;
  const int ty = t2 / tiles_x;
  t.ty0 = ty * kRTH;
  t.tx0 = (t2 - ty * tiles_x) * kRTW;
  return t;
}

typedef __attribute__((address_space(1))) char gchar_t;
typedef __attribute__((ext_vector_type(4))) unsigned u32x4_t;
typedef __attribute__((ext_vector_type(4))) float f32x4_t;
typedef __attribute__((address_space(1))) u32x4_t guint4_t;
typedef __attribute__((address_space(1))) f32x4_t gfloat4_t;
__device__ __forceinline__ void gstore(gchar_t* p, uint4 v) { *reinterpret_cast<guint4_t*>(p) = u32x4_t{v.x, v.y, v.z, v.w}; }
__device__ __forceinline__ void gstore(gchar_t* p, float4 v) { *reinterpret_cast<gfloat4_t*>(p) = f32x4_t{v.x, v.y, v.z, v.w}; }
__device__ __forceinline__ uint4 gload_u4(const gchar_t* p) { const u32x4_t v = *reinterpret_cast<const guint4_t*>(p); return make_uint4(v.x, v.y, v.z, v.w); }
__device__ __forceinline__ float4 gload_f4(const gchar_t* p) { const f32x4_t v = *reinterpret_cast<const gfloat4_t*>(p); return make_float4(v.x, v.y, v.z, v.w); }
__device__ __forceinline__ gchar_t* tab_ptr(const int* T, int lo) {
  return reinterpret_cast<gchar_t*>(((unsigned long long)(unsigned)T[lo + 1] << 32) | (unsigned)T[lo]);
}

__device__ __forceinline__ void glds16(const void* src, unsigned lds_off) {
  unsigned keep;
  asm volatile("s_mov_b32 %0, m0\n\ts_mov_b32 m0, %2\n\ts_nop 0\n\tglobal_load_lds_dwordx4 %1, off\n\ts_mov_b32 m0, %0"
               : "=&s"(keep) : "v"(src), "s"(lds_off) : "memory");
}

__device__ __forceinline__ void res_stage(const int* tabL, const void* zeros, const ResTile& t, int ch, unsigned xoff, int wq, int lane) {
  const int* T = tabL + t.gi * 32;
  const char* sbase = (const char*)(tab_ptr(T, kTSrcLo) + (long long)t.b * T[kTSrcSb2] + ch * 128);
  const int sy2 = T[kTSrcSy2], sx2 = T[kTSrcSx2];
  const int H = T[kTH], W = T[kTW];
  const int sub = lane >> 3, cl = lane & 7;
#pragma unroll
  for (int i = 0; i < (kRNG + 3) / 4; ++i) {
    const int g = wq + 4 * i;
    if (i * 4 + 3 < kRNG || g < kRNG) {
      const int p = g * 8 + sub;
      const int hy = __mul24(p, 241) >> 13;
      const int hx = p - __mul24(hy, kRHW);
      const int iy = t.ty0 - 1 + hy, ix = t.tx0 - 1 + hx;
      const int c = cl ^ ((hx >> 1) & 7);
      const bool ok = (p < kRNHP) && ((unsigned)iy < (unsigned)H) && ((unsigned)ix < (unsigned)W);
      const int off = __mul24(iy, sy2) + __mul24(ix, sx2) + c * 16;
      const char* src = ok ? sbase + off : reinterpret_cast<const char*>(zeros);
      glds16(src, __builtin_amdgcn_readfirstlane(xoff + g * 1024));
    }
  }
}

#define FCVSR_RES_STAMP(SLOT)                                                                                          \
  do {                                                                                                                 \
    if (a.stamps && blockIdx.x == 8 && p < 64 && lane == 0)                                                            \
      a.stamps[(wave * 64 + p) * 8 + (SLOT)] = __builtin_amdgcn_s_memtime();                                           \
  } while (0)

template <bool BF16, int MODE, int NCH, int NSU>
__global__ __launch_bounds__(512, 2) void conv3_res_kernel(ResK a) {
  constexpr bool DST16 = MODE != 0;
  constexpr bool FAST = MODE == 2;
  extern __shared__ __align__(16) unsigned char lds[];
  constexpr int CO = 64 / NCH;
  constexpr int MF = CO / 32;
  const int tid = threadIdx.x;
  const int lane = tid & 63, wave = __builtin_amdgcn_readfirstlane(tid >> 6);
  const int r = lane & 31, h = lane >> 5;
  const int grp = wave >> 2, wq = wave & 3;
  const unsigned lds0 = (unsigned)(uintptr_t)(__attribute__((address_space(3))) void*)lds;

  const int NB = a.cout / CO;
  const int xcd = blockIdx.x & 7, loc = blockIdx.x >> 3;
  const int nb = loc % NB, slot = loc / NB, nslots = (gridDim.x >> 3) / NB;
  const int tb = (int)((long long)xcd * a.total_tiles / 8), te = (int)((long long)(xcd + 1) * a.total_tiles / 8);
  const int n0 = nb * CO;
  const int ntile = (tb + slot < te) ? (te - tb - slot + nslots - 1) / nslots : 0;
  if (ntile == 0) return;
  const int nmine = (ntile - grp + 1) >> 1;
  const int NU = nmine * NCH;
  const int plast = 2 * ((ntile + 1) >> 1) * NCH;

  {
    const int sub = lane >> 3, cl = lane & 7;
#pragma unroll
    for (int i = 0; i < kRWRows / 8 / 8; ++i) {
      const int g = wave + 8 * i;
      const int row = g * 8 + sub;
      const int q = row / CO, co = row - q * CO;
      const int ch = q / 9, tap = q - ch * 9;
      const int c = cl ^ ((co >> 1) & 7);
      const uint16_t* src = a.w + ((long long)tap * a.cout_pad + n0 + co) * a.cin_pad + ch * 64 + c * 8;
      glds16(src, __builtin_amdgcn_readfirstlane(lds0 + g * 1024));
    }
  }
  if (tid < CO) reinterpret_cast<float*>(lds + kRBiasOff)[tid] = a.bias ? a.bias[n0 + tid] : 0.f;
  if (tid >= 128 && tid < 128 + 96) reinterpret_cast<int*>(lds + kRTabOff)[tid - 128] = a.tab[(tid - 128) >> 5][(tid - 128) & 31];
  const int* tabL = reinterpret_cast<const int*>(lds + kRTabOff);
  const unsigned xoff = lds0 + kRWBytes + grp * kRXBytes;
  __syncthreads();
  ResTile tcur = res_decode(tabL, a.n_groups, tb + slot + grp * nslots < te ? tb + slot + grp * nslots : tb + slot);
  if (grp == 0 && !(a.dbg & 1)) res_stage(tabL, a.zeros, tcur, 0, xoff, wq, lane);

  float ns = 1.f;
  if (a.act == FCVSR_ACT_RELU) ns = 0.f;
  else if (a.act == FCVSR_ACT_LEAKY) ns = a.slope;
  else if (a.act == FCVSR_ACT_PRELU) ns = *reinterpret_cast<const __attribute__((address_space(1))) float*>(reinterpret_cast<uintptr_t>(a.slope_ptr));
  const bool r16 = a.res16 != 0;

  unsigned wb[4], xb[3][4];
#pragma unroll
  for (int kk = 0; kk < 4; ++kk) {
    wb[kk] = r * 128 + (((2 * kk + h) ^ ((r >> 1) & 7)) << 4);
#pragma unroll
    for (int kx = 0; kx < 3; ++kx)
      xb[kx][kk] = kRWBytes + grp * kRXBytes + (2 * wq * kRHW + r + kx) * 128 + (((2 * kk + h) ^ (((r + kx) >> 1) & 7)) << 4);
  }

  f32x16_t acc[MF][2];
  asm volatile("s_waitcnt vmcnt(0)" ::: "memory");
  __syncthreads();

  int k = 0;
#pragma unroll 1
  for (int p = 0;; ++p) {
    FCVSR_RES_STAMP(0);
    if ((p & 1) == grp) {
      if (k < NU) {
        const int ch = (NCH == 1) ? 0 : (k & (NCH - 1));
        if (ch == 0) {
#pragma unroll
          for (int mf = 0; mf < MF; ++mf)
#pragma unroll
            for (int j = 0; j < 2; ++j)
#pragma unroll
              for (int i = 0; i < 16; ++i) acc[mf][j][i] = 0.f;
        }
        if (!(a.dbg & 2)) {
          __builtin_amdgcn_s_setprio(2);
          const unsigned wch = ch * (9 * CO * 128);
          uint4 wf[3][MF], xf[3][2];
#define FCVSR_RES_LOAD(S, SLOT)                                                                                  \
  do {                                                                                                           \
    constexpr int tap_ = (S) / 4, kk_ = (S) % 4, ky_ = tap_ / 3, kx_ = tap_ % 3;                                 \
    _Pragma("unroll") for (int mf = 0; mf < MF; ++mf)                                                            \
        wf[SLOT][mf] = *reinterpret_cast<const uint4*>(lds + wb[kk_] + wch + (tap_ * CO + mf * 32) * 128);       \
    _Pragma("unroll") for (int j = 0; j < 2; ++j)                                                                \
        xf[SLOT][j] = *reinterpret_cast<const uint4*>(lds + xb[kx_][kk_] + (j + ky_) * kRRowB);                   \
  } while (0)
#define FCVSR_RES_STEP(S)                                                                                        \
  do {                                                                                                           \
    if ((S) + 2 < 36) FCVSR_RES_LOAD(((S) + 2) % 36, ((S) + 2) % 3);                                             \
    _Pragma("unroll") for (int mf = 0; mf < MF; ++mf)                                                            \
        _Pragma("unroll") for (int j = 0; j < 2; ++j)                                                            \
            acc[mf][j] = mfma<BF16>(wf[(S) % 3][mf], xf[(S) % 3][j], acc[mf][j]);                                 \
    if ((S) + 2 < 36) __builtin_amdgcn_sched_group_barrier(0x100, MF + 2, 0);                                    \
    __builtin_amdgcn_sched_group_barrier(0x008, 2 * MF, 0);                                                      \
  } while (0)
          FCVSR_RES_LOAD(0, 0);
          FCVSR_RES_LOAD(1, 1);
          __builtin_amdgcn_sched_barrier(0);
          FCVSR_RES_STEP(0);  FCVSR_RES_STEP(1);  FCVSR_RES_STEP(2);  FCVSR_RES_STEP(3);  FCVSR_RES_STEP(4);  FCVSR_RES_STEP(5);
          FCVSR_RES_STEP(6);  FCVSR_RES_STEP(7);  FCVSR_RES_STEP(8);  FCVSR_RES_STEP(9);  FCVSR_RES_STEP(10); FCVSR_RES_STEP(11);
          FCVSR_RES_STEP(12); FCVSR_RES_STEP(13); FCVSR_RES_STEP(14); FCVSR_RES_STEP(15); FCVSR_RES_STEP(16); FCVSR_RES_STEP(17);
          FCVSR_RES_STEP(18); FCVSR_RES_STEP(19); FCVSR_RES_STEP(20); FCVSR_RES_STEP(21); FCVSR_RES_STEP(22); FCVSR_RES_STEP(23);
          FCVSR_RES_STEP(24); FCVSR_RES_STEP(25); FCVSR_RES_STEP(26); FCVSR_RES_STEP(27); FCVSR_RES_STEP(28); FCVSR_RES_STEP(29);
          FCVSR_RES_STEP(30); FCVSR_RES_STEP(31); FCVSR_RES_STEP(32); FCVSR_RES_STEP(33); FCVSR_RES_STEP(34); FCVSR_RES_STEP(35);
#undef FCVSR_RES_STEP
#undef FCVSR_RES_LOAD
          __builtin_amdgcn_s_setprio(0);
        }
        FCVSR_RES_STAMP(1);
        if (ch == NCH - 1 && !(a.dbg & 8)) {
          const float* bias_a = reinterpret_cast<const float*>(lds + kRBiasOff) + 4 * h;
#pragma unroll
          for (int mf = 0; mf < MF; ++mf)
#pragma unroll
            for (int j = 0; j < 2; ++j)
#pragma unroll
              for (int g = 0; g < 4; ++g) {
                const float4 b4 = *reinterpret_cast<const float4*>(bias_a + mf * 32 + 8 * g);
                float v[4] = {acc[mf][j][4 * g] + b4.x, acc[mf][j][4 * g + 1] + b4.y, acc[mf][j][4 * g + 2] + b4.z,
                              acc[mf][j][4 * g + 3] + b4.w};
#pragma unroll
                for (int e = 0; e < 4; ++e)
                  if (NSU != 2) v[e] = NSU == 1 ? fmaxf(v[e], ns * v[e]) : fmaxf(v[e], 0.f) + ns * fminf(v[e], 0.f);
                if (FAST) {
                  const uint2 pk = cvt4<BF16>(make_float4(v[0], v[1], v[2], v[3]));
                  acc[mf][j][2 * g] = __uint_as_float(pk.x);
                  acc[mf][j][2 * g + 1] = __uint_as_float(pk.y);
                } else {
#pragma unroll
                  for (int e = 0; e < 4; ++e) acc[mf][j][4 * g + e] = v[e];
                }
              }
        }
      }
      ++k;
      asm volatile("s_waitcnt lgkmcnt(0)" ::: "memory");
      FCVSR_RES_STAMP(2);
    } else {
      ResTile tn = tcur;
      if (k < NU) {
        const int ch = (NCH == 1) ? 0 : (k & (NCH - 1));
        if (ch == 0 && k > 0) tn = res_decode(tabL, a.n_groups, tb + slot + (2 * (k / NCH) + grp) * nslots);
        if (!(a.dbg & 1)) res_stage(tabL, a.zeros, tn, ch, xoff, wq, lane);
      }
      FCVSR_RES_STAMP(3);
      int nst = 0;
      if (k >= 1 && k <= NU && ((k - 1) & (NCH - 1)) == NCH - 1 && !(a.dbg & 8)) {
        const ResTile t = tcur;
        const int* T = tabL + t.gi * 32;
        const int GH = T[kTH], GW = T[kTW];
        gchar_t* dbase = tab_ptr(T, kTDstLo);
        const gchar_t* r0base = tab_ptr(T, kTR0Lo);
        const gchar_t* r1base = tab_ptr(T, kTR1Lo);
        const int px = t.tx0 + r;
#pragma unroll
        for (int j = 0; j < 2; ++j) {
          if (j) __builtin_amdgcn_sched_barrier(0);
          const int py = t.ty0 + 2 * wq + j;
          const bool ok = (py < GH) && (px < GW) && !(a.dbg & 4);
          const int pyc = ok ? py : 0, pxc = ok ? px : 0;
          const int cq4 = a.cout >> 2, sp = a.ps ? n0 / cq4 : 0, nch = a.ps ? n0 - sp * cq4 : n0;
          const int dyy = a.ps ? 2 * pyc + (sp >> 1) : pyc, dxx = a.ps ? 2 * pxc + (sp & 1) : pxc;
          const unsigned dpix = (unsigned)(t.b * T[kTDstSb] + dyy * T[kTDstSy] + dxx * T[kTDstSx] + nch + 8 * h);
          const unsigned r0pix = (unsigned)(t.b * T[kTR0Sb] + pyc * T[kTR0Sy] + pxc * T[kTR0Sx] + n0 + 8 * h);
          const unsigned r1pix = (unsigned)(t.b * T[kTR1Sb] + pyc * T[kTR1Sy] + pxc * T[kTR1Sx] + n0 + 8 * h);
          if (FAST) {
            if (__builtin_amdgcn_ballot_w64(ok) != 0) nst += MF * 2;
#pragma unroll
            for (int mf = 0; mf < MF; ++mf)
#pragma unroll
              for (int q = 0; q < 2; ++q) {
                typedef __attribute__((ext_vector_type(2))) unsigned u2_t;
                const u2_t s0 = __builtin_amdgcn_permlane32_swap(__float_as_uint(acc[mf][j][4 * q]), __float_as_uint(acc[mf][j][4 * q + 2]), false, false);
                const u2_t s1 = __builtin_amdgcn_permlane32_swap(__float_as_uint(acc[mf][j][4 * q + 1]), __float_as_uint(acc[mf][j][4 * q + 3]), false, false);
                if (ok) gstore(dbase + (size_t)(dpix + mf * 32 + 16 * q) * 2, make_uint4(s0.x, s1.x, s0.y, s1.y));
              }
            continue;
          }
          float x[MF][2][8];
#pragma unroll
          for (int mf = 0; mf < MF; ++mf)
#pragma unroll
            for (int q = 0; q < 2; ++q)
#pragma unroll
              for (int e = 0; e < 4; ++e) {
                typedef __attribute__((ext_vector_type(2))) unsigned u2_t;
                const u2_t sw = __builtin_amdgcn_permlane32_swap(__float_as_uint(acc[mf][j][8 * q + e]),
                                                                 __float_as_uint(acc[mf][j][8 * q + 4 + e]), false, false);
                x[mf][q][e] = __uint_as_float(sw.x);
                x[mf][q][4 + e] = __uint_as_float(sw.y);
              }
#pragma unroll
          for (int ri = 0; ri < 2; ++ri) {
            if (ri < a.n_res) {
              const gchar_t* rp = ri == 0 ? r0base : r1base;
              const unsigned rpix = ri == 0 ? r0pix : r1pix;
              const float rs = a.rs[ri];
              if (r16) {
                uint4 v[MF][2];
#pragma unroll
                for (int mf = 0; mf < MF; ++mf)
#pragma unroll
                  for (int q = 0; q < 2; ++q)
                    v[mf][q] = gload_u4(rp + (size_t)(rpix + mf * 32 + 16 * q) * 2);
#pragma unroll
                for (int mf = 0; mf < MF; ++mf)
#pragma unroll
                  for (int q = 0; q < 2; ++q) {
                    float rr[8];
                    cvt16x4_to_f32<BF16>(make_uint2(v[mf][q].x, v[mf][q].y), rr);
                    cvt16x4_to_f32<BF16>(make_uint2(v[mf][q].z, v[mf][q].w), rr + 4);
#pragma unroll
                    for (int e = 0; e < 8; ++e) x[mf][q][e] = fmaf(rs, rr[e], x[mf][q][e]);
                  }
              } else {
                float4 v[MF][2][2];
#pragma unroll
                for (int mf = 0; mf < MF; ++mf)
#pragma unroll
                  for (int q = 0; q < 2; ++q) {
                    v[mf][q][0] = gload_f4(rp + (size_t)(rpix + mf * 32 + 16 * q) * 4);
                    v[mf][q][1] = gload_f4(rp + (size_t)(rpix + mf * 32 + 16 * q + 4) * 4);
                  }
#pragma unroll
                for (int mf = 0; mf < MF; ++mf)
#pragma unroll
                  for (int q = 0; q < 2; ++q) {
                    const float4 u0 = v[mf][q][0], u1 = v[mf][q][1];
                    x[mf][q][0] = fmaf(rs, u0.x, x[mf][q][0]); x[mf][q][1] = fmaf(rs, u0.y, x[mf][q][1]);
                    x[mf][q][2] = fmaf(rs, u0.z, x[mf][q][2]); x[mf][q][3] = fmaf(rs, u0.w, x[mf][q][3]);
                    x[mf][q][4] = fmaf(rs, u1.x, x[mf][q][4]); x[mf][q][5] = fmaf(rs, u1.y, x[mf][q][5]);
                    x[mf][q][6] = fmaf(rs, u1.z, x[mf][q][6]); x[mf][q][7] = fmaf(rs, u1.w, x[mf][q][7]);
                  }
              }
            }
          }
          if (__builtin_amdgcn_ballot_w64(ok) != 0) nst += MF * 2 * (DST16 ? 1 : 2);
          if (ok) {
#pragma unroll
            for (int mf = 0; mf < MF; ++mf)
#pragma unroll
              for (int q = 0; q < 2; ++q) {
                const float* xx = x[mf][q];
                if (DST16) {
                  const uint2 lo = cvt4<BF16>(make_float4(xx[0], xx[1], xx[2], xx[3])), hi = cvt4<BF16>(make_float4(xx[4], xx[5], xx[6], xx[7]));
                  gstore(dbase + (size_t)(dpix + mf * 32 + 16 * q) * 2, make_uint4(lo.x, lo.y, hi.x, hi.y));
                } else {
                  gstore(dbase + (size_t)(dpix + mf * 32 + 16 * q) * 4, make_float4(xx[0], xx[1], xx[2], xx[3]));
                  gstore(dbase + (size_t)(dpix + mf * 32 + 16 * q + 4) * 4, make_float4(xx[4], xx[5], xx[6], xx[7]));
                }
              }
          }
        }
      }
      tcur = tn;
      FCVSR_RES_STAMP(4);
      constexpr int SR = MF * 2 * (DST16 ? 1 : 2);
      if (nst == 0) asm volatile("s_waitcnt vmcnt(0)" ::: "memory");
      else if (nst == SR) asm volatile("s_waitcnt vmcnt(%0)" ::"n"(SR) : "memory");
      else asm volatile("s_waitcnt vmcnt(%0)" ::"n"(2 * SR) : "memory");
      FCVSR_RES_STAMP(5);
    }
    FCVSR_RES_STAMP(6);
    __builtin_amdgcn_s_barrier();
    if (p >= plast) break;
  }
}


template <bool BF16, int NCH, int NSU, int PF>
__global__ __launch_bounds__(768, 3) void conv3_res3_kernel(ResK a) {
  extern __shared__ __align__(16) unsigned char lds[];
  constexpr int CO = 64 / NCH;
  constexpr int MF = CO / 32;
  const int tid = threadIdx.x;
  const int lane = tid & 63, wave = __builtin_amdgcn_readfirstlane(tid >> 6);
  const int grp = wave >> 2, wq = wave & 3;
  const unsigned lds0 = (unsigned)(uintptr_t)(__attribute__((address_space(3))) void*)lds;

  const int NB = a.cout / CO;
  const int xcd = blockIdx.x & 7, loc = blockIdx.x >> 3;
  const int nb = loc % NB, slot = loc / NB, nslots = (gridDim.x >> 3) / NB;
  const int tb = (int)((long long)xcd * a.total_tiles / 8), te = (int)((long long)(xcd + 1) * a.total_tiles / 8);
  const int n0 = nb * CO;
  const int ntile = (tb + slot < te) ? (te - tb - slot + nslots - 1) / nslots : 0;
  if (ntile == 0) return;
  const int nmine = ntile > grp ? (ntile - grp + 2) / 3 : 0;
  const int TMAX = (ntile + 2) / 3;

  {
    const int sub = lane >> 3, cl = lane & 7;
#pragma unroll
    for (int i = 0; i < kRWRows / 8 / 12; ++i) {
      const int g = wave + 12 * i;
      const int row = g * 8 + sub;
      const int q = row / CO, co = row - q * CO;
      const int ch = q / 9, tap = q - ch * 9;
      const int c = cl ^ ((co >> 1) & 7);
      const int co_src = (co & ~31) | (((co >> 2) & 1) << 4) | (((co >> 3) & 3) << 2) | (co & 3);
      const uint16_t* src = a.w + ((long long)tap * a.cout_pad + n0 + co_src) * a.cin_pad + ch * 64 + c * 8;
      glds16(src, __builtin_amdgcn_readfirstlane(lds0 + g * 1024));
    }
  }
  if (tid < CO) reinterpret_cast<float*>(lds + kRBiasOff)[tid] = a.bias ? a.bias[n0 + tid] : 0.f;
  if (tid >= 128 && tid < 128 + 96) reinterpret_cast<int*>(lds + kRTabOff)[tid - 128] = a.tab[(tid - 128) >> 5][(tid - 128) & 31];
  const int* tabL = reinterpret_cast<const int*>(lds + kRTabOff);

  float ns = 1.f;
  if (a.act == FCVSR_ACT_RELU) ns = 0.f;
  else if (a.act == FCVSR_ACT_LEAKY) ns = a.slope;
  else if (a.act == FCVSR_ACT_PRELU) ns = *reinterpret_cast<const __attribute__((address_space(1))) float*>(reinterpret_cast<uintptr_t>(a.slope_ptr));

  asm volatile("s_waitcnt vmcnt(0)" ::: "memory");
  __syncthreads();

  for (int i = 0; i < grp; ++i) __builtin_amdgcn_s_barrier();
#pragma unroll 1
  for (int ti = 0; ti < TMAX; ++ti) {
    const bool act = ti < nmine;
    int lv = lane, z0 = 0;
    asm volatile("" : "+v"(lv), "+s"(z0));
    const int r = lv & 31, h = lv >> 5;
    const int* tabP = tabL + z0;
    const int tile = tb + slot + (3 * ti + grp) * nslots;
    f32x16_t acc[MF][2];
#pragma unroll
    for (int ch = 0; ch < NCH; ++ch) {
      const int p0 = grp + 3 * (ti * NCH + ch);
      const unsigned bsel = ((p0 + 1) & 1) * kRXBytes;
      if (act) {
        if (!(a.dbg & 1)) {
          if (!(a.dbg & 16)) __builtin_amdgcn_s_setprio(1);
          const ResTile t = res_decode(tabP, a.n_groups, tile);
          res_stage(tabP, a.zeros, t, ch, lds0 + kRWBytes + bsel, wq, lv);
          __builtin_amdgcn_s_setprio(0);
        }
        asm volatile("s_waitcnt vmcnt(0)" ::: "memory");
      }
      __builtin_amdgcn_s_barrier();
      if (act) {
        if (ch == 0) {
#pragma unroll
          for (int mf = 0; mf < MF; ++mf)
#pragma unroll
            for (int j = 0; j < 2; ++j)
#pragma unroll
              for (int i = 0; i < 16; ++i) acc[mf][j][i] = 0.f;
        }
        if (!(a.dbg & 2)) {
          if (a.dbg & 64) __builtin_amdgcn_s_setprio(3); else __builtin_amdgcn_s_setprio(2);
          const unsigned wch = ch * (9 * CO * 128);
          const unsigned xsel = kRWBytes + bsel;
          unsigned wb[4], xb[3][4];
#pragma unroll
          for (int kk = 0; kk < 4; ++kk) {
            wb[kk] = wch + r * 128 + (((2 * kk + h) ^ ((r >> 1) & 7)) << 4);
#pragma unroll
            for (int kx = 0; kx < 3; ++kx)
              xb[kx][kk] = xsel + (2 * wq * kRHW + r + kx) * 128 + (((2 * kk + h) ^ (((r + kx) >> 1) & 7)) << 4);
          }
          uint4 wf[PF][MF], xf[PF][2];
#define FCVSR_RES_LOAD(S, SLOT)                                                                                  \
  do {                                                                                                           \
    constexpr int tap_ = (S) / 4, kk_ = (S) % 4, ky_ = tap_ / 3, kx_ = tap_ % 3;                                 \
    _Pragma("unroll") for (int mf = 0; mf < MF; ++mf)                                                            \
        wf[SLOT][mf] = *reinterpret_cast<const uint4*>(lds + wb[kk_] + (tap_ * CO + mf * 32) * 128);             \
    _Pragma("unroll") for (int j = 0; j < 2; ++j)                                                                \
        xf[SLOT][j] = *reinterpret_cast<const uint4*>(lds + xb[kx_][kk_] + (j + ky_) * kRRowB);                   \
  } while (0)
#define FCVSR_RES_STEP(S)                                                                                        \
  do {                                                                                                           \
    if ((S) + PF - 1 < 36) FCVSR_RES_LOAD(((S) + PF - 1) % 36, ((S) + PF - 1) % PF);                             \
    _Pragma("unroll") for (int mf = 0; mf < MF; ++mf)                                                            \
        _Pragma("unroll") for (int j = 0; j < 2; ++j)                                                            \
            acc[mf][j] = mfma<BF16>(wf[(S) % PF][mf], xf[(S) % PF][j], acc[mf][j]);                               \
    if ((S) + PF - 1 < 36) __builtin_amdgcn_sched_group_barrier(0x100, MF + 2, 0);                               \
    __builtin_amdgcn_sched_group_barrier(0x008, 2 * MF, 0);                                                      \
  } while (0)
          FCVSR_RES_LOAD(0, 0);
          FCVSR_RES_LOAD(1, 1);
          if (PF > 3) FCVSR_RES_LOAD(2, 2);
          __builtin_amdgcn_sched_barrier(0);
          FCVSR_RES_STEP(0);  FCVSR_RES_STEP(1);  FCVSR_RES_STEP(2);  FCVSR_RES_STEP(3);  FCVSR_RES_STEP(4);  FCVSR_RES_STEP(5);
          FCVSR_RES_STEP(6);  FCVSR_RES_STEP(7);  FCVSR_RES_STEP(8);  FCVSR_RES_STEP(9);  FCVSR_RES_STEP(10); FCVSR_RES_STEP(11);
          FCVSR_RES_STEP(12); FCVSR_RES_STEP(13); FCVSR_RES_STEP(14); FCVSR_RES_STEP(15); FCVSR_RES_STEP(16); FCVSR_RES_STEP(17);
          FCVSR_RES_STEP(18); FCVSR_RES_STEP(19); FCVSR_RES_STEP(20); FCVSR_RES_STEP(21); FCVSR_RES_STEP(22); FCVSR_RES_STEP(23);
          FCVSR_RES_STEP(24); FCVSR_RES_STEP(25); FCVSR_RES_STEP(26); FCVSR_RES_STEP(27); FCVSR_RES_STEP(28); FCVSR_RES_STEP(29);
          FCVSR_RES_STEP(30); FCVSR_RES_STEP(31); FCVSR_RES_STEP(32); FCVSR_RES_STEP(33); FCVSR_RES_STEP(34); FCVSR_RES_STEP(35);
#undef FCVSR_RES_STEP
#undef FCVSR_RES_LOAD
          __builtin_amdgcn_s_setprio(0);
        }
        asm volatile("s_waitcnt lgkmcnt(0)" ::: "memory");
      }
      __builtin_amdgcn_s_barrier();
      if (act && ch == NCH - 1 && !(a.dbg & 8)) {
        if (a.dbg & 32) __builtin_amdgcn_s_setprio(1);
        const ResTile t = res_decode(tabP, a.n_groups, tile);
        const int* T = tabP + t.gi * 32;
        const int GH = T[kTH], GW = T[kTW];
        gchar_t* dbase = tab_ptr(T, kTDstLo);
        const int px = t.tx0 + r;
        const float* bias_a = reinterpret_cast<const float*>(lds + kRBiasOff) + 16 * h;
        const int cq4 = a.cout >> 2, sp = a.ps ? n0 / cq4 : 0, nch = a.ps ? n0 - sp * cq4 : n0;
#pragma unroll
        for (int j = 0; j < 2; ++j) {
          uint2 pk[MF][4];
#pragma unroll
          for (int mf = 0; mf < MF; ++mf)
#pragma unroll
            for (int g = 0; g < 4; ++g) {
              const float4 b4 = *reinterpret_cast<const float4*>(bias_a + mf * 32 + 4 * g);
              float v[4] = {acc[mf][j][4 * g] + b4.x, acc[mf][j][4 * g + 1] + b4.y, acc[mf][j][4 * g + 2] + b4.z,
                            acc[mf][j][4 * g + 3] + b4.w};
#pragma unroll
              for (int e = 0; e < 4; ++e)
                if (NSU != 2) v[e] = NSU == 1 ? fmaxf(v[e], ns * v[e]) : fmaxf(v[e], 0.f) + ns * fminf(v[e], 0.f);
              pk[mf][g] = cvt4<BF16>(make_float4(v[0], v[1], v[2], v[3]));
            }
          const int py = t.ty0 + 2 * wq + j;
          const bool ok = (py < GH) && (px < GW) && !(a.dbg & 4);
          const int pyc = ok ? py : 0, pxc = ok ? px : 0;
          const int dyy = a.ps ? 2 * pyc + (sp >> 1) : pyc, dxx = a.ps ? 2 * pxc + (sp & 1) : pxc;
          const unsigned dpix = (unsigned)(t.b * T[kTDstSb] + dyy * T[kTDstSy] + dxx * T[kTDstSx] + nch + 16 * h);
          if (ok) {
#pragma unroll
            for (int mf = 0; mf < MF; ++mf)
#pragma unroll
              for (int q = 0; q < 2; ++q)
                gstore(dbase + (size_t)(dpix + mf * 32 + 8 * q) * 2, make_uint4(pk[mf][2 * q].x, pk[mf][2 * q].y, pk[mf][2 * q + 1].x, pk[mf][2 * q + 1].y));
          }
        }
      }
      __builtin_amdgcn_s_barrier();
    }
  }
  for (int i = 0; i < 2 - grp; ++i) __builtin_amdgcn_s_barrier();
}

bool conv3_res_supports(int cin, int cout) { return (cin == 64 && cout % 64 == 0) || (cin == 128 && cout % 32 == 0); }

template <bool BF16, int MODE, int NCH, int NSU>
static hipError_t launch_res(const ResArgs& a, hipStream_t st) {
  static DevOnce attr;
  int dev = 0;
  hipError_t e = once_per_device(attr, [&] {
    hipError_t e1 = hipFuncSetAttribute((const void*)conv3_res_kernel<BF16, MODE, NCH, NSU>, hipFuncAttributeMaxDynamicSharedMemorySize, (int)kRLds);
    if constexpr (BF16 && MODE == 2)
      if (e1 == hipSuccess)
        e1 = hipFuncSetAttribute((const void*)conv3_res3_kernel<true, NCH, NSU, 3>, hipFuncAttributeMaxDynamicSharedMemorySize, (int)kRLds);
    return e1;
  }, &dev);
  if (e != hipSuccess) return e;
  const int cus = device_cu_count(dev);
  if (cus <= 0) return hipErrorInvalidDevice;
  int n_cu = cus > 8 ? cus / 8 * 8 : 8;
  {
    static const int lim = getenv("FCVSR_RES_CUS") ? atoi(getenv("FCVSR_RES_CUS")) : 0;
    if (lim >= 8 && lim < n_cu) n_cu = lim / 8 * 8;
  }
  const int NB = a.cout / (64 / NCH);
  int grid = n_cu / (8 * NB) * (8 * NB);
  if (grid < 8 * NB) grid = 8 * NB;
  const int need = (a.total_tiles + 7) / 8 * 8 * NB;
  if (grid > need) grid = need;
  ResK k;
  k.n_groups = a.n_groups; k.total_tiles = a.total_tiles; k.cout = a.cout; k.cout_pad = a.cout_pad; k.cin_pad = a.cin_pad;
  k.act = a.act; k.n_res = a.n_res; k.res16 = a.res16; k.dbg = a.dbg; k.ps = a.ps; k.slope = a.slope; k.rs[0] = a.rs[0]; k.rs[1] = a.rs[1];
  k.slope_ptr = a.slope_ptr; k.w = a.w; k.bias = a.bias; k.zeros = a.zeros; k.stamps = a.stamps;
  for (int g = 0; g < 3; ++g) {
    const ResGroup& G = a.g[g < a.n_groups ? g : 0];
    int* T = k.tab[g];
    for (int i = 0; i < 32; ++i) T[i] = 0;
    auto put = [&](int lo, const void* p) { T[lo] = (int)(unsigned)((uintptr_t)p & 0xffffffffu); T[lo + 1] = (int)(unsigned)((uintptr_t)p >> 32); };
    put(kTSrcLo, G.src.p);
    T[kTSrcSb2] = (int)(G.src.sb * 2); T[kTSrcSy2] = (int)(G.src.sy * 2); T[kTSrcSx2] = (int)(G.src.sx * 2);
    T[kTH] = G.H; T[kTW] = G.W; T[kTTilesX] = G.tiles_x; T[kTPerImg] = G.tiles_x * G.tiles_y;
    T[kTTileBegin] = g < a.n_groups ? G.tile_begin : 0x7fffffff;
    put(kTDstLo, G.dst.p); T[kTDstSb] = (int)G.dst.sb; T[kTDstSy] = (int)G.dst.sy; T[kTDstSx] = (int)G.dst.sx;
    const View& r0 = a.n_res > 0 ? G.res[0] : G.dst;
    const View& r1 = a.n_res > 1 ? G.res[1] : G.dst;
    put(kTR0Lo, r0.p); T[kTR0Sb] = (int)r0.sb; T[kTR0Sy] = (int)r0.sy; T[kTR0Sx] = (int)r0.sx;
    put(kTR1Lo, r1.p); T[kTR1Sb] = (int)r1.sb; T[kTR1Sy] = (int)r1.sy; T[kTR1Sx] = (int)r1.sx;
  }
  bool v2 = false;
  if constexpr (BF16 && MODE == 2) {
    if (a.variant == 3) {
      hipLaunchKernelGGL((conv3_res3_kernel<true, NCH, NSU, 3>), dim3(grid), dim3(768), kRLds, st, k);
      v2 = true;
    }
  }
  if (!v2) hipLaunchKernelGGL((conv3_res_kernel<BF16, MODE, NCH, NSU>), dim3(grid), dim3(512), kRLds, st, k);
  return hipGetLastError();
}

template <bool BF16, int NCH>
static hipError_t launch_res_mode(const ResArgs& a, bool dst16, hipStream_t st) {
  const bool nsu = a.act == FCVSR_ACT_NONE || a.act == FCVSR_ACT_RELU || (a.act == FCVSR_ACT_LEAKY && a.slope >= 0.f && a.slope <= 1.f);
  const int mode = !dst16 ? 0 : (a.n_res == 0 ? 2 : 1);
  if (a.act == FCVSR_ACT_NONE) {
    if (mode == 0) return launch_res<BF16, 0, NCH, 2>(a, st);
    if (mode == 1) return launch_res<BF16, 1, NCH, 2>(a, st);
    return launch_res<BF16, 2, NCH, 2>(a, st);
  }
  if (nsu) {
    if (mode == 0) return launch_res<BF16, 0, NCH, 1>(a, st);
    if (mode == 1) return launch_res<BF16, 1, NCH, 1>(a, st);
    return launch_res<BF16, 2, NCH, 1>(a, st);
  }
  if (mode == 0) return launch_res<BF16, 0, NCH, 0>(a, st);
  if (mode == 1) return launch_res<BF16, 1, NCH, 0>(a, st);
  return launch_res<BF16, 2, NCH, 0>(a, st);
}

hipError_t launch_conv3_res(const ResArgs& a, bool bf16, bool dst16, hipStream_t st) {
  if (!conv3_res_supports(a.cin, a.cout)) return hipErrorInvalidValue;
  if (a.cin == 64) return bf16 ? launch_res_mode<true, 1>(a, dst16, st) : launch_res_mode<false, 1>(a, dst16, st);
  return bf16 ? launch_res_mode<true, 2>(a, dst16, st) : launch_res_mode<false, 2>(a, dst16, st);
}

}
```

### fcvsr_amd/csrc/mfma_util.h

```cpp
#pragma once
#include "common.h"

namespace fcvsr {

typedef __attribute__((ext_vector_type(8))) __bf16 bf16x8_t;
typedef __attribute__((ext_vector_type(8))) _Float16 f16x8_t;
typedef __attribute__((ext_vector_type(4))) __bf16 bf16x4_t;
typedef __attribute__((ext_vector_type(4))) _Float16 f16x4_t;
typedef __attribute__((ext_vector_type(16))) float f32x16_t;


template <bool BF16>
__device__ __forceinline__ uint2 cvt4(float4 v) {
  if (BF16) {
    bf16x4_t c = {(__bf16)v.x, (__bf16)v.y, (__bf16)v.z, (__bf16)v.w};
    return __builtin_bit_cast(uint2, c);
  } else {
    f16x4_t c = {(_Float16)v.x, (_Float16)v.y, (_Float16)v.z, (_Float16)v.w};
    return __builtin_bit_cast(uint2, c);
  }
}

template <bool BF16>
__device__ __forceinline__ f32x16_t mfma(uint4 a, uint4 b, f32x16_t c) {
  if (BF16)
    return __builtin_amdgcn_mfma_f32_32x32x16_bf16(__builtin_bit_cast(bf16x8_t, a), __builtin_bit_cast(bf16x8_t, b), c, 0, 0, 0);
  else
    return __builtin_amdgcn_mfma_f32_32x32x16_f16(__builtin_bit_cast(f16x8_t, a), __builtin_bit_cast(f16x8_t, b), c, 0, 0, 0);
}

template <bool BF16>
__device__ __forceinline__ void cvt16x4_to_f32(uint2 v, float* o) {
  if (BF16) {
    o[0] = __uint_as_float(v.x << 16); o[1] = __uint_as_float(v.x & 0xffff0000u);
    o[2] = __uint_as_float(v.y << 16); o[3] = __uint_as_float(v.y & 0xffff0000u);
  } else {
    typedef __attribute__((ext_vector_type(2))) _Float16 h2;
    const h2 a = __builtin_bit_cast(h2, v.x), b = __builtin_bit_cast(h2, v.y);
    o[0] = (float)a[0]; o[1] = (float)a[1]; o[2] = (float)b[0]; o[3] = (float)b[1];
  }
}

template <bool BF16, int NV>
__device__ __forceinline__ void load_res(const float* base, long long off, bool r16, float* o) {
  if (r16) {
    const uint16_t* p = reinterpret_cast<const uint16_t*>(base) + off;
    if (NV == 8) {
      const uint4 v = *reinterpret_cast<const uint4*>(p);
      cvt16x4_to_f32<BF16>(make_uint2(v.x, v.y), o);
      cvt16x4_to_f32<BF16>(make_uint2(v.z, v.w), o + 4);
    } else {
      cvt16x4_to_f32<BF16>(*reinterpret_cast<const uint2*>(p), o);
    }
  } else {
#pragma unroll
    for (int k = 0; k < NV; k += 4) {
      const float4 t = *reinterpret_cast<const float4*>(base + off + k);
      o[k] = t.x; o[k + 1] = t.y; o[k + 2] = t.z; o[k + 3] = t.w;
    }
  }
}

}
```

Baseline: 824.3.

## Switch resident-weight conv to 16x16x32 MFMA and drop the variant-3 kernel

Rewrites the resident-weight 3x3 conv inner loop to use 16x16x32 MFMA tiles instead of 32x32x16. This changes the LDS swizzle, the fragment addressing, the accumulator layout and the epilogue, which now uses permlane16 swaps. The scheduling hints interleave single LDS reads with MFMAs. It also deletes the experimental conv3_res3 kernel and its env-var variant selector. The goal is better MFMA/LDS interleaving and lower accumulator register pressure, at the cost of more MFMA instructions and a new data layout that could introduce bank conflicts.

Measured after the change: 849.7 (median of 6 runs). 3.1% higher.

```diff
diff --git a/fcvsr_amd/csrc/conv_mfma.hip b/fcvsr_amd/csrc/conv_mfma.hip
--- a/fcvsr_amd/csrc/conv_mfma.hip
+++ b/fcvsr_amd/csrc/conv_mfma.hip
@@ -1360,7 +1360,6 @@
     wa.w = a.w; wa.bias = a.bias; wa.act = a.act; wa.slope = a.slope; wa.slope_ptr = a.slope_ptr;
     wa.rs[0] = a.rs[0]; wa.rs[1] = a.rs[1]; wa.n_res = a.n_res; wa.res16 = a.res16; wa.ps = a.ps; wa.zeros = zeros;
     { const char* wd_ = getenv("FCVSR_RES_DBG"); wa.dbg = wd_ ? atoi(wd_) : 0; }
-    { const char* wv_ = getenv("FCVSR_RES_V"); wa.variant = wv_ ? atoi(wv_) : 1; }
     wa.stamps = nullptr;
     {
       const char* ws_ = getenv("FCVSR_RES_STAMPS");
@@ -1370,7 +1369,7 @@
         wa.stamps = (unsigned long long*)g_res_stamps;
       }
     }
-    FCVSR_NOTE_KERNEL((wa.variant >= 3 && mma_dtype == FCVSR_BF16 && a.dst16 && a.n_res == 0) ? "conv3_res3_kernel<%s, %d, %d, %d>" : "conv3_res_kernel<%s, %d, %d, %d>", tf(mma_dtype == FCVSR_BF16), !a.dst16 ? 0 : (a.n_res == 0 ? 2 : 1), cin / 64,
+    FCVSR_NOTE_KERNEL("conv3_res_kernel<%s, %d, %d, %d>", tf(mma_dtype == FCVSR_BF16), !a.dst16 ? 0 : (a.n_res == 0 ? 2 : 1), cin / 64,
                       a.act == FCVSR_ACT_NONE ? 2 : ((a.act == FCVSR_ACT_RELU || (a.act == FCVSR_ACT_LEAKY && a.slope >= 0.f && a.slope <= 1.f)) ? 1 : 0));
     e = launch_conv3_res(wa, mma_dtype == FCVSR_BF16, a.dst16 != 0, st);
     if (e != hipSuccess) {
diff --git a/fcvsr_amd/csrc/conv_res.h b/fcvsr_amd/csrc/conv_res.h
--- a/fcvsr_amd/csrc/conv_res.h
+++ b/fcvsr_amd/csrc/conv_res.h
@@ -25,7 +25,6 @@
   int n_res, res16;
   int ps;
   const void* zeros;
-  int variant;
   int dbg;
   unsigned long long* stamps;
 };
diff --git a/fcvsr_amd/csrc/conv_res.hip b/fcvsr_amd/csrc/conv_res.hip
--- a/fcvsr_amd/csrc/conv_res.hip
+++ b/fcvsr_amd/csrc/conv_res.hip
@@ -15,6 +15,8 @@
 constexpr int kRBiasOff = kRWBytes + 2 * kRXBytes;
 constexpr int kRTabOff = kRBiasOff + 256;
 constexpr size_t kRLds = (size_t)kRTabOff + 3 * 32 * 4;
+
+__device__ __forceinline__ int res_swz(int x) { return ((x >> 1) & 3) | ((x << 1) & 4); }
 
 enum {
   kTSrcLo = 0, kTSrcHi, kTSrcSb2, kTSrcSy2, kTSrcSx2, kTH, kTW, kTTilesX, kTPerImg, kTTileBegin,
@@ -54,7 +56,6 @@
 
 typedef __attribute__((address_space(1))) char gchar_t;
 typedef __attribute__((ext_vector_type(4))) unsigned u32x4_t;
-typedef __attribute__((ext_vector_type(4))) float f32x4_t;
 typedef __attribute__((address_space(1))) u32x4_t guint4_t;
 typedef __attribute__((address_space(1))) f32x4_t gfloat4_t;
 __device__ __forceinline__ void gstore(gchar_t* p, uint4 v) { *reinterpret_cast<guint4_t*>(p) = u32x4_t{v.x, v.y, v.z, v.w}; }
@@ -85,7 +86,7 @@
       const int hy = __mul24(p, 241) >> 13;
       const int hx = p - __mul24(hy, kRHW);
       const int iy = t.ty0 - 1 + hy, ix = t.tx0 - 1 + hx;
-      const int c = cl ^ ((hx >> 1) & 7);
+      const int c = cl ^ res_swz(hx);
       const bool ok = (p < kRNHP) && ((unsigned)iy < (unsigned)H) && ((unsigned)ix < (unsigned)W);
       const int off = __mul24(iy, sy2) + __mul24(ix, sx2) + c * 16;
       const char* src = ok ? sbase + off : reinterpret_cast<const char*>(zeros);
@@ -109,7 +110,6 @@
   constexpr int MF = CO / 32;
   const int tid = threadIdx.x;
   const int lane = tid & 63, wave = __builtin_amdgcn_readfirstlane(tid >> 6);
-  const int r = lane & 31, h = lane >> 5;
   const int grp = wave >> 2, wq = wave & 3;
   const unsigned lds0 = (unsigned)(uintptr_t)(__attribute__((address_space(3))) void*)lds;
 
@@ -132,7 +132,7 @@
       const int row = g * 8 + sub;
       const int q = row / CO, co = row - q * CO;
       const int ch = q / 9, tap = q - ch * 9;
-      const int c = cl ^ ((co >> 1) & 7);
+      const int c = cl ^ res_swz(co);
       const uint16_t* src = a.w + ((long long)tap * a.cout_pad + n0 + co) * a.cin_pad + ch * 64 + c * 8;
       glds16(src, __builtin_amdgcn_readfirstlane(lds0 + g * 1024));
     }
@@ -151,16 +151,17 @@
   else if (a.act == FCVSR_ACT_PRELU) ns = *reinterpret_cast<const __attribute__((address_space(1))) float*>(reinterpret_cast<uintptr_t>(a.slope_ptr));
   const bool r16 = a.res16 != 0;
 
-  unsigned wb[4], xb[3][4];
-#pragma unroll
-  for (int kk = 0; kk < 4; ++kk) {
-    wb[kk] = r * 128 + (((2 * kk + h) ^ ((r >> 1) & 7)) << 4);
+  const int p16 = lane & 15, G = lane >> 4;
+  constexpr int MF16 = CO / 16;
+  unsigned wb[2], xb[3][2];
+#pragma unroll
+  for (int ks = 0; ks < 2; ++ks) {
+    wb[ks] = p16 * 128 + (((4 * ks + G) ^ res_swz(p16)) << 4);
 #pragma unroll
     for (int kx = 0; kx < 3; ++kx)
-      xb[kx][kk] = kRWBytes + grp * kRXBytes + (2 * wq * kRHW + r + kx) * 128 + (((2 * kk + h) ^ (((r + kx) >> 1) & 7)) << 4);
-  }
-
-  f32x16_t acc[MF][2];
+      xb[kx][ks] = kRWBytes + grp * kRXBytes + (2 * wq * kRHW + p16 + kx) * 128 + (((4 * ks + G) ^ res_swz(p16 + kx)) << 4);
+  }
+  f32x4_t acc[MF16][4];
   asm volatile("s_waitcnt vmcnt(0)" ::: "memory");
   __syncthreads();
 
@@ -173,32 +174,38 @@
         const int ch = (NCH == 1) ? 0 : (k & (NCH - 1));
         if (ch == 0) {
 #pragma unroll
-          for (int mf = 0; mf < MF; ++mf)
-#pragma unroll
-            for (int j = 0; j < 2; ++j)
-#pragma unroll
-              for (int i = 0; i < 16; ++i) acc[mf][j][i] = 0.f;
+          for (int mf = 0; mf < MF16; ++mf)
+#pragma unroll
+            for (int nf = 0; nf < 4; ++nf) acc[mf][nf] = f32x4_t{0.f, 0.f, 0.f, 0.f};
         }
         if (!(a.dbg & 2)) {
           __builtin_amdgcn_s_setprio(2);
           const unsigned wch = ch * (9 * CO * 128);
-          uint4 wf[3][MF], xf[3][2];
+          uint4 wf[3][MF16], xf[3][4];
 #define FCVSR_RES_LOAD(S, SLOT)                                                                                  \
   do {                                                                                                           \
-    constexpr int tap_ = (S) / 4, kk_ = (S) % 4, ky_ = tap_ / 3, kx_ = tap_ % 3;                                 \
-    _Pragma("unroll") for (int mf = 0; mf < MF; ++mf)                                                            \
-        wf[SLOT][mf] = *reinterpret_cast<const uint4*>(lds + wb[kk_] + wch + (tap_ * CO + mf * 32) * 128);       \
-    _Pragma("unroll") for (int j = 0; j < 2; ++j)                                                                \
-        xf[SLOT][j] = *reinterpret_cast<const uint4*>(lds + xb[kx_][kk_] + (j + ky_) * kRRowB);                   \
+    constexpr int tap_ = (S) / 2, ks_ = (S) % 2, ky_ = tap_ / 3, kx_ = tap_ % 3;                                 \
+    _Pragma("unroll") for (int mf = 0; mf < MF16; ++mf)                                                          \
+        wf[SLOT][mf] = *reinterpret_cast<const uint4*>(lds + wb[ks_] + wch + (tap_ * CO + mf * 16) * 128);       \
+    _Pragma("unroll") for (int nf = 0; nf < 4; ++nf)                                                             \
+        xf[SLOT][nf] = *reinterpret_cast<const uint4*>(lds + xb[kx_][ks_] + ((nf >> 1) + ky_) * kRRowB + (nf & 1) * 2048); \
   } while (0)
 #define FCVSR_RES_STEP(S)                                                                                        \
   do {                                                                                                           \
-    if ((S) + 2 < 36) FCVSR_RES_LOAD(((S) + 2) % 36, ((S) + 2) % 3);                                             \
-    _Pragma("unroll") for (int mf = 0; mf < MF; ++mf)                                                            \
-        _Pragma("unroll") for (int j = 0; j < 2; ++j)                                                            \
-            acc[mf][j] = mfma<BF16>(wf[(S) % 3][mf], xf[(S) % 3][j], acc[mf][j]);                                 \
-    if ((S) + 2 < 36) __builtin_amdgcn_sched_group_barrier(0x100, MF + 2, 0);                                    \
-    __builtin_amdgcn_sched_group_barrier(0x008, 2 * MF, 0);                                                      \
+    if ((S) + 2 < 18) FCVSR_RES_LOAD(((S) + 2) % 18, ((S) + 2) % 3);                                             \
+    _Pragma("unroll") for (int mf = 0; mf < MF16; ++mf)                                                          \
+        _Pragma("unroll") for (int nf = 0; nf < 4; ++nf)                                                         \
+            acc[mf][nf] = mfma16x16x32<BF16>(wf[(S) % 3][mf], xf[(S) % 3][nf], acc[mf][nf]);                      \
+    if ((S) + 2 < 18) {                                                                                          \
+      _Pragma("unroll") for (int i_ = 0; i_ < MF16 + 4; ++i_) {                                                  \
+        __builtin_amdgcn_sched_group_barrier(0x008, 4 * MF16 / (MF16 + 4), 0);                                   \
+        __builtin_amdgcn_sched_group_barrier(0x100, 1, 0);                                                       \
+      }                                                                                                          \
+      if (4 * MF16 > (MF16 + 4) * (4 * MF16 / (MF16 + 4)))                                                       \
+        __builtin_amdgcn_sched_group_barrier(0x008, 4 * MF16 - (MF16 + 4) * (4 * MF16 / (MF16 + 4)), 0);         \
+    } else {                                                                                                     \
+      __builtin_amdgcn_sched_group_barrier(0x008, 4 * MF16, 0);                                                  \
+    }                                                                                                            \
   } while (0)
           FCVSR_RES_LOAD(0, 0);
           FCVSR_RES_LOAD(1, 1);
@@ -206,37 +213,32 @@
           FCVSR_RES_STEP(0);  FCVSR_RES_STEP(1);  FCVSR_RES_STEP(2);  FCVSR_RES_STEP(3);  FCVSR_RES_STEP(4);  FCVSR_RES_STEP(5);
           FCVSR_RES_STEP(6);  FCVSR_RES_STEP(7);  FCVSR_RES_STEP(8);  FCVSR_RES_STEP(9);  FCVSR_RES_STEP(10); FCVSR_RES_STEP(11);
           FCVSR_RES_STEP(12); FCVSR_RES_STEP(13); FCVSR_RES_STEP(14); FCVSR_RES_STEP(15); FCVSR_RES_STEP(16); FCVSR_RES_STEP(17);
-          FCVSR_RES_STEP(18); FCVSR_RES_STEP(19); FCVSR_RES_STEP(20); FCVSR_RES_STEP(21); FCVSR_RES_STEP(22); FCVSR_RES_STEP(23);
-          FCVSR_RES_STEP(24); FCVSR_RES_STEP(25); FCVSR_RES_STEP(26); FCVSR_RES_STEP(27); FCVSR_RES_STEP(28); FCVSR_RES_STEP(29);
-          FCVSR_RES_STEP(30); FCVSR_RES_STEP(31); FCVSR_RES_STEP(32); FCVSR_RES_STEP(33); FCVSR_RES_STEP(34); FCVSR_RES_STEP(35);
 #undef FCVSR_RES_STEP
 #undef FCVSR_RES_LOAD
           __builtin_amdgcn_s_setprio(0);
         }
         FCVSR_RES_STAMP(1);
         if (ch == NCH - 1 && !(a.dbg & 8)) {
-          const float* bias_a = reinterpret_cast<const float*>(lds + kRBiasOff) + 4 * h;
-#pragma unroll
-          for (int mf = 0; mf < MF; ++mf)
-#pragma unroll
-            for (int j = 0; j < 2; ++j)
-#pragma unroll
-              for (int g = 0; g < 4; ++g) {
-                const float4 b4 = *reinterpret_cast<const float4*>(bias_a + mf * 32 + 8 * g);
-                float v[4] = {acc[mf][j][4 * g] + b4.x, acc[mf][j][4 * g + 1] + b4.y, acc[mf][j][4 * g + 2] + b4.z,
-                              acc[mf][j][4 * g + 3] + b4.w};
-#pragma unroll
-                for (int e = 0; e < 4; ++e)
-                  if (NSU != 2) v[e] = NSU == 1 ? fmaxf(v[e], ns * v[e]) : fmaxf(v[e], 0.f) + ns * fminf(v[e], 0.f);
-                if (FAST) {
-                  const uint2 pk = cvt4<BF16>(make_float4(v[0], v[1], v[2], v[3]));
-                  acc[mf][j][2 * g] = __uint_as_float(pk.x);
-                  acc[mf][j][2 * g + 1] = __uint_as_float(pk.y);
-                } else {
-#pragma unroll
-                  for (int e = 0; e < 4; ++e) acc[mf][j][4 * g + e] = v[e];
-                }
+          const float* bias_a = reinterpret_cast<const float*>(lds + kRBiasOff) + 4 * G;
+#pragma unroll
+          for (int mf = 0; mf < MF16; ++mf) {
+            const float4 b4 = *reinterpret_cast<const float4*>(bias_a + mf * 16);
+#pragma unroll
+            for (int nf = 0; nf < 4; ++nf) {
+              float v[4] = {acc[mf][nf][0] + b4.x, acc[mf][nf][1] + b4.y, acc[mf][nf][2] + b4.z, acc[mf][nf][3] + b4.w};
+#pragma unroll
+              for (int e = 0; e < 4; ++e)
+                if (NSU != 2) v[e] = NSU == 1 ? fmaxf(v[e], ns * v[e]) : fmaxf(v[e], 0.f) + ns * fminf(v[e], 0.f);
+              if (FAST) {
+                const uint2 pk = cvt4<BF16>(make_float4(v[0], v[1], v[2], v[3]));
+                acc[mf][nf][0] = __uint_as_float(pk.x);
+                acc[mf][nf][1] = __uint_as_float(pk.y);
+              } else {
+#pragma unroll
+                for (int e = 0; e < 4; ++e) acc[mf][nf][e] = v[e];
               }
+            }
+          }
         }
       }
       ++k;
@@ -258,113 +260,117 @@
         gchar_t* dbase = tab_ptr(T, kTDstLo);
         const gchar_t* r0base = tab_ptr(T, kTR0Lo);
         const gchar_t* r1base = tab_ptr(T, kTR1Lo);
-        const int px = t.tx0 + r;
+        const int cl8 = 16 * (G & 1) + 8 * (G >> 1);
+        const int cq4 = a.cout >> 2, sp = a.ps ? n0 / cq4 : 0, nch = a.ps ? n0 - sp * cq4 : n0;
+        typedef __attribute__((ext_vector_type(2))) unsigned u2_t;
 #pragma unroll
         for (int j = 0; j < 2; ++j) {
           if (j) __builtin_amdgcn_sched_barrier(0);
           const int py = t.ty0 + 2 * wq + j;
-          const bool ok = (py < GH) && (px < GW) && !(a.dbg & 4);
-          const int pyc = ok ? py : 0, pxc = ok ? px : 0;
-          const int cq4 = a.cout >> 2, sp = a.ps ? n0 / cq4 : 0, nch = a.ps ? n0 - sp * cq4 : n0;
-          const int dyy = a.ps ? 2 * pyc + (sp >> 1) : pyc, dxx = a.ps ? 2 * pxc + (sp & 1) : pxc;
-          const unsigned dpix = (unsigned)(t.b * T[kTDstSb] + dyy * T[kTDstSy] + dxx * T[kTDstSx] + nch + 8 * h);
-          const unsigned r0pix = (unsigned)(t.b * T[kTR0Sb] + pyc * T[kTR0Sy] + pxc * T[kTR0Sx] + n0 + 8 * h);
-          const unsigned r1pix = (unsigned)(t.b * T[kTR1Sb] + pyc * T[kTR1Sy] + pxc * T[kTR1Sx] + n0 + 8 * h);
+          bool ok[2];
+          unsigned dpix[2], rpix[2][2];
+#pragma unroll
+          for (int hf = 0; hf < 2; ++hf) {
+            const int px = t.tx0 + 16 * hf + p16;
+            ok[hf] = (py < GH) && (px < GW) && !(a.dbg & 4);
+            const int pyc = ok[hf] ? py : 0, pxc = ok[hf] ? px : 0;
+            const int dyy = a.ps ? 2 * pyc + (sp >> 1) : pyc, dxx = a.ps ? 2 * pxc + (sp & 1) : pxc;
+            dpix[hf] = (unsigned)(t.b * T[kTDstSb] + dyy * T[kTDstSy] + dxx * T[kTDstSx] + nch + cl8);
+            rpix[0][hf] = (unsigned)(t.b * T[kTR0Sb] + pyc * T[kTR0Sy] + pxc * T[kTR0Sx] + n0 + cl8);
+            rpix[1][hf] = (unsigned)(t.b * T[kTR1Sb] + pyc * T[kTR1Sy] + pxc * T[kTR1Sx] + n0 + cl8);
+            if (__builtin_amdgcn_ballot_w64(ok[hf]) != 0) nst += MF * (DST16 ? 1 : 2);
+          }
           if (FAST) {
-            if (__builtin_amdgcn_ballot_w64(ok) != 0) nst += MF * 2;
-#pragma unroll
-            for (int mf = 0; mf < MF; ++mf)
-#pragma unroll
-              for (int q = 0; q < 2; ++q) {
-                typedef __attribute__((ext_vector_type(2))) unsigned u2_t;
-                const u2_t s0 = __builtin_amdgcn_permlane32_swap(__float_as_uint(acc[mf][j][4 * q]), __float_as_uint(acc[mf][j][4 * q + 2]), false, false);
-                const u2_t s1 = __builtin_amdgcn_permlane32_swap(__float_as_uint(acc[mf][j][4 * q + 1]), __float_as_uint(acc[mf][j][4 * q + 3]), false, false);
-                if (ok) gstore(dbase + (size_t)(dpix + mf * 32 + 16 * q) * 2, make_uint4(s0.x, s1.x, s0.y, s1.y));
+#pragma unroll
+            for (int hf = 0; hf < 2; ++hf)
+#pragma unroll
+              for (int m = 0; m < MF; ++m) {
+                const int nf = 2 * j + hf;
+                const u2_t s0 = __builtin_amdgcn_permlane16_swap(__float_as_uint(acc[2 * m][nf][0]), __float_as_uint(acc[2 * m + 1][nf][0]), false, false);
+                const u2_t s1 = __builtin_amdgcn_permlane16_swap(__float_as_uint(acc[2 * m][nf][1]), __float_as_uint(acc[2 * m + 1][nf][1]), false, false);
+                if (ok[hf]) gstore(dbase + (size_t)(dpix[hf] + 32 * m) * 2, make_uint4(s0.x, s1.x, s0.y, s1.y));
               }
             continue;
           }
-          float x[MF][2][8];
-#pragma unroll
-          for (int mf = 0; mf < MF; ++mf)
-#pragma unroll
-            for (int q = 0; q < 2; ++q)
+          float x[2][MF][8];
+#pragma unroll
+          for (int hf = 0; hf < 2; ++hf)
+#pragma unroll
+            for (int m = 0; m < MF; ++m)
 #pragma unroll
               for (int e = 0; e < 4; ++e) {
-                typedef __attribute__((ext_vector_type(2))) unsigned u2_t;
-                const u2_t sw = __builtin_amdgcn_permlane32_swap(__float_as_uint(acc[mf][j][8 * q + e]),
-                                                                 __float_as_uint(acc[mf][j][8 * q + 4 + e]), false, false);
-                x[mf][q][e] = __uint_as_float(sw.x);
-                x[mf][q][4 + e] = __uint_as_float(sw.y);
+                const int nf = 2 * j + hf;
+                const u2_t sw = __builtin_amdgcn_permlane16_swap(__float_as_uint(acc[2 * m][nf][e]), __float_as_uint(acc[2 * m + 1][nf][e]), false, false);
+                x[hf][m][e] = __uint_as_float(sw.x);
+                x[hf][m][4 + e] = __uint_as_float(sw.y);
               }
 #pragma unroll
           for (int ri = 0; ri < 2; ++ri) {
             if (ri < a.n_res) {
               const gchar_t* rp = ri == 0 ? r0base : r1base;
-              const unsigned rpix = ri == 0 ? r0pix : r1pix;
               const float rs = a.rs[ri];
               if (r16) {
-                uint4 v[MF][2];
-#pragma unroll
-                for (int mf = 0; mf < MF; ++mf)
-#pragma unroll
-                  for (int q = 0; q < 2; ++q)
-                    v[mf][q] = gload_u4(rp + (size_t)(rpix + mf * 32 + 16 * q) * 2);
-#pragma unroll
-                for (int mf = 0; mf < MF; ++mf)
-#pragma unroll
-                  for (int q = 0; q < 2; ++q) {
+                uint4 v[2][MF];
+#pragma unroll
+                for (int hf = 0; hf < 2; ++hf)
+#pragma unroll
+                  for (int m = 0; m < MF; ++m) v[hf][m] = gload_u4(rp + (size_t)(rpix[ri][hf] + 32 * m) * 2);
+#pragma unroll
+                for (int hf = 0; hf < 2; ++hf)
+#pragma unroll
+                  for (int m = 0; m < MF; ++m) {
                     float rr[8];
-                    cvt16x4_to_f32<BF16>(make_uint2(v[mf][q].x, v[mf][q].y), rr);
-                    cvt16x4_to_f32<BF16>(make_uint2(v[mf][q].z, v[mf][q].w), rr + 4);
-#pragma unroll
-                    for (int e = 0; e < 8; ++e) x[mf][q][e] = fmaf(rs, rr[e], x[mf][q][e]);
+                    cvt16x4_to_f32<BF16>(make_uint2(v[hf][m].x, v[hf][m].y), rr);
+                    cvt16x4_to_f32<BF16>(make_uint2(v[hf][m].z, v[hf][m].w), rr + 4);
+#pragma unroll
+                    for (int e = 0; e < 8; ++e) x[hf][m][e] = fmaf(rs, rr[e], x[hf][m][e]);
                   }
               } else {
-                float4 v[MF][2][2];
-#pragma unroll
-                for (int mf = 0; mf < MF; ++mf)
-#pragma unroll
-                  for (int q = 0; q < 2; ++q) {
-                    v[mf][q][0] = gload_f4(rp + (size_t)(rpix + mf * 32 + 16 * q) * 4);
-                    v[mf][q][1] = gload_f4(rp + (size_t)(rpix + mf * 32 + 16 * q + 4) * 4);
+                float4 v[2][MF][2];
+#pragma unroll
+                for (int hf = 0; hf < 2; ++hf)
+#pragma unroll
+                  for (int m = 0; m < MF; ++m) {
+                    v[hf][m][0] = gload_f4(rp + (size_t)(rpix[ri][hf] + 32 * m) * 4);
+                    v[hf][m][1] = gload_f4(rp + (size_t)(rpix[ri][hf] + 32 * m + 4) * 4);
                   }
 #pragma unroll
-                for (int mf = 0; mf < MF; ++mf)
-#pragma unroll
-                  for (int q = 0; q < 2; ++q) {
-                    const float4 u0 = v[mf][q][0], u1 = v[mf][q][1];
-                    x[mf][q][0] = fmaf(rs, u0.x, x[mf][q][0]); x[mf][q][1] = fmaf(rs, u0.y, x[mf][q][1]);
-                    x[mf][q][2] = fmaf(rs, u0.z, x[mf][q][2]); x[mf][q][3] = fmaf(rs, u0.w, x[mf][q][3]);
-                    x[mf][q][4] = fmaf(rs, u1.x, x[mf][q][4]); x[mf][q][5] = fmaf(rs, u1.y, x[mf][q][5]);
-                    x[mf][q][6] = fmaf(rs, u1.z, x[mf][q][6]); x[mf][q][7] = fmaf(rs, u1.w, x[mf][q][7]);
+                for (int hf = 0; hf < 2; ++hf)
+#pragma unroll
+                  for (int m = 0; m < MF; ++m) {
+                    const float4 u0 = v[hf][m][0], u1 = v[hf][m][1];
+                    float* xx = x[hf][m];
+                    xx[0] = fmaf(rs, u0.x, xx[0]); xx[1] = fmaf(rs, u0.y, xx[1]); xx[2] = fmaf(rs, u0.z, xx[2]); xx[3] = fmaf(rs, u0.w, xx[3]);
+                    xx[4] = fmaf(rs, u1.x, xx[4]); xx[5] = fmaf(rs, u1.y, xx[5]); xx[6] = fmaf(rs, u1.z, xx[6]); xx[7] = fmaf(rs, u1.w, xx[7]);
                   }
               }
             }
           }
-          if (__builtin_amdgcn_ballot_w64(ok) != 0) nst += MF * 2 * (DST16 ? 1 : 2);
-          if (ok) {
-#pragma unroll
-            for (int mf = 0; mf < MF; ++mf)
-#pragma unroll
-              for (int q = 0; q < 2; ++q) {
-                const float* xx = x[mf][q];
+#pragma unroll
+          for (int hf = 0; hf < 2; ++hf)
+            if (ok[hf]) {
+#pragma unroll
+              for (int m = 0; m < MF; ++m) {
+                const float* xx = x[hf][m];
                 if (DST16) {
                   const uint2 lo = cvt4<BF16>(make_float4(xx[0], xx[1], xx[2], xx[3])), hi = cvt4<BF16>(make_float4(xx[4], xx[5], xx[6], xx[7]));
-                  gstore(dbase + (size_t)(dpix + mf * 32 + 16 * q) * 2, make_uint4(lo.x, lo.y, hi.x, hi.y));
+                  gstore(dbase + (size_t)(dpix[hf] + 32 * m) * 2, make_uint4(lo.x, lo.y, hi.x, hi.y));
                 } else {
-                  gstore(dbase + (size_t)(dpix + mf * 32 + 16 * q) * 4, make_float4(xx[0], xx[1], xx[2], xx[3]));
-                  gstore(dbase + (size_t)(dpix + mf * 32 + 16 * q + 4) * 4, make_float4(xx[4], xx[5], xx[6], xx[7]));
+                  gstore(dbase + (size_t)(dpix[hf] + 32 * m) * 4, make_float4(xx[0], xx[1], xx[2], xx[3]));
+                  gstore(dbase + (size_t)(dpix[hf] + 32 * m + 4) * 4, make_float4(xx[4], xx[5], xx[6], xx[7]));
                 }
               }
-          }
+            }
         }
       }
       tcur = tn;
       FCVSR_RES_STAMP(4);
-      constexpr int SR = MF * 2 * (DST16 ? 1 : 2);
+      constexpr int SH = MF * (DST16 ? 1 : 2);
       if (nst == 0) asm volatile("s_waitcnt vmcnt(0)" ::: "memory");
-      else if (nst == SR) asm volatile("s_waitcnt vmcnt(%0)" ::"n"(SR) : "memory");
-      else asm volatile("s_waitcnt vmcnt(%0)" ::"n"(2 * SR) : "memory");
+      else if (nst == SH) asm volatile("s_waitcnt vmcnt(%0)" ::"n"(SH) : "memory");
+      else if (nst == 2 * SH) asm volatile("s_waitcnt vmcnt(%0)" ::"n"(2 * SH) : "memory");
+      else if (nst == 3 * SH) asm volatile("s_waitcnt vmcnt(%0)" ::"n"(3 * SH) : "memory");
+      else asm volatile("s_waitcnt vmcnt(%0)" ::"n"(4 * SH) : "memory");
       FCVSR_RES_STAMP(5);
     }
     FCVSR_RES_STAMP(6);
@@ -374,176 +380,6 @@
 }
 
 
-template <bool BF16, int NCH, int NSU, int PF>
-__global__ __launch_bounds__(768, 3) void conv3_res3_kernel(ResK a) {
-  extern __shared__ __align__(16) unsigned char lds[];
-  constexpr int CO = 64 / NCH;
-  constexpr int MF = CO / 32;
-  const int tid = threadIdx.x;
-  const int lane = tid & 63, wave = __builtin_amdgcn_readfirstlane(tid >> 6);
-  const int grp = wave >> 2, wq = wave & 3;
-  const unsigned lds0 = (unsigned)(uintptr_t)(__attribute__((address_space(3))) void*)lds;
-
-  const int NB = a.cout / CO;
-  const int xcd = blockIdx.x & 7, loc = blockIdx.x >> 3;
-  const int nb = loc % NB, slot = loc / NB, nslots = (gridDim.x >> 3) / NB;
-  const int tb = (int)((long long)xcd * a.total_tiles / 8), te = (int)((long long)(xcd + 1) * a.total_tiles / 8);
-  const int n0 = nb * CO;
-  const int ntile = (tb + slot < te) ? (te - tb - slot + nslots - 1) / nslots : 0;
-  if (ntile == 0) return;
-  const int nmine = ntile > grp ? (ntile - grp + 2) / 3 : 0;
-  const int TMAX = (ntile + 2) / 3;
-
-  {
-    const int sub = lane >> 3, cl = lane & 7;
-#pragma unroll
-    for (int i = 0; i < kRWRows / 8 / 12; ++i) {
-      const int g = wave + 12 * i;
-      const int row = g * 8 + sub;
-      const int q = row / CO, co = row - q * CO;
-      const int ch = q / 9, tap = q - ch * 9;
-      const int c = cl ^ ((co >> 1) & 7);
-      const int co_src = (co & ~31) | (((co >> 2) & 1) << 4) | (((co >> 3) & 3) << 2) | (co & 3);
-      const uint16_t* src = a.w + ((long long)tap * a.cout_pad + n0 + co_src) * a.cin_pad + ch * 64 + c * 8;
-      glds16(src, __builtin_amdgcn_readfirstlane(lds0 + g * 1024));
-    }
-  }
-  if (tid < CO) reinterpret_cast<float*>(lds + kRBiasOff)[tid] = a.bias ? a.bias[n0 + tid] : 0.f;
-  if (tid >= 128 && tid < 128 + 96) reinterpret_cast<int*>(lds + kRTabOff)[tid - 128] = a.tab[(tid - 128) >> 5][(tid - 128) & 31];
-  const int* tabL = reinterpret_cast<const int*>(lds + kRTabOff);
-
-  float ns = 1.f;
-  if (a.act == FCVSR_ACT_RELU) ns = 0.f;
-  else if (a.act == FCVSR_ACT_LEAKY) ns = a.slope;
-  else if (a.act == FCVSR_ACT_PRELU) ns = *reinterpret_cast<const __attribute__((address_space(1))) float*>(reinterpret_cast<uintptr_t>(a.slope_ptr));
-
-  asm volatile("s_waitcnt vmcnt(0)" ::: "memory");
-  __syncthreads();
-
-  for (int i = 0; i < grp; ++i) __builtin_amdgcn_s_barrier();
-#pragma unroll 1
-  for (int ti = 0; ti < TMAX; ++ti) {
-    const bool act = ti < nmine;
-    int lv = lane, z0 = 0;
-    asm volatile("" : "+v"(lv), "+s"(z0));
-    const int r = lv & 31, h = lv >> 5;
-    const int* tabP = tabL + z0;
-    const int tile = tb + slot + (3 * ti + grp) * nslots;
-    f32x16_t acc[MF][2];
-#pragma unroll
-    for (int ch = 0; ch < NCH; ++ch) {
-      const int p0 = grp + 3 * (ti * NCH + ch);
-      const unsigned bsel = ((p0 + 1) & 1) * kRXBytes;
-      if (act) {
-        if (!(a.dbg & 1)) {
-          if (!(a.dbg & 16)) __builtin_amdgcn_s_setprio(1);
-          const ResTile t = res_decode(tabP, a.n_groups, tile);
-          res_stage(tabP, a.zeros, t, ch, lds0 + kRWBytes + bsel, wq, lv);
-          __builtin_amdgcn_s_setprio(0);
-        }
-        asm volatile("s_waitcnt vmcnt(0)" ::: "memory");
-      }
-      __builtin_amdgcn_s_barrier();
-      if (act) {
-        if (ch == 0) {
-#pragma unroll
-          for (int mf = 0; mf < MF; ++mf)
-#pragma unroll
-            for (int j = 0; j < 2; ++j)
-#pragma unroll
-              for (int i = 0; i < 16; ++i) acc[mf][j][i] = 0.f;
-        }
-        if (!(a.dbg & 2)) {
-          if (a.dbg & 64) __builtin_amdgcn_s_setprio(3); else __builtin_amdgcn_s_setprio(2);
-          const unsigned wch = ch * (9 * CO * 128);
-          const unsigned xsel = kRWBytes + bsel;
-          unsigned wb[4], xb[3][4];
-#pragma unroll
-          for (int kk = 0; kk < 4; ++kk) {
-            wb[kk] = wch + r * 128 + (((2 * kk + h) ^ ((r >> 1) & 7)) << 4);
-#pragma unroll
-            for (int kx = 0; kx < 3; ++kx)
-              xb[kx][kk] = xsel + (2 * wq * kRHW + r + kx) * 128 + (((2 * kk + h) ^ (((r + kx) >> 1) & 7)) << 4);
-          }
-          uint4 wf[PF][MF], xf[PF][2];
-#define FCVSR_RES_LOAD(S, SLOT)                                                                                  \
-  do {                                                                                                           \
-    constexpr int tap_ = (S) / 4, kk_ = (S) % 4, ky_ = tap_ / 3, kx_ = tap_ % 3;                                 \
-    _Pragma("unroll") for (int mf = 0; mf < MF; ++mf)                                                            \
-        wf[SLOT][mf] = *reinterpret_cast<const uint4*>(lds + wb[kk_] + (tap_ * CO + mf * 32) * 128);             \
-    _Pragma("unroll") for (int j = 0; j < 2; ++j)                                                                \
-        xf[SLOT][j] = *reinterpret_cast<const uint4*>(lds + xb[kx_][kk_] + (j + ky_) * kRRowB);                   \
-  } while (0)
-#define FCVSR_RES_STEP(S)                                                                                        \
-  do {                                                                                                           \
-    if ((S) + PF - 1 < 36) FCVSR_RES_LOAD(((S) + PF - 1) % 36, ((S) + PF - 1) % PF);                             \
-    _Pragma("unroll") for (int mf = 0; mf < MF; ++mf)                                                            \
-        _Pragma("unroll") for (int j = 0; j < 2; ++j)                                                            \
-            acc[mf][j] = mfma<BF16>(wf[(S) % PF][mf], xf[(S) % PF][j], acc[mf][j]);                               \
-    if ((S) + PF - 1 < 36) __builtin_amdgcn_sched_group_barrier(0x100, MF + 2, 0);                               \
-    __builtin_amdgcn_sched_group_barrier(0x008, 2 * MF, 0);                                                      \
-  } while (0)
-          FCVSR_RES_LOAD(0, 0);
-          FCVSR_RES_LOAD(1, 1);
-          if (PF > 3) FCVSR_RES_LOAD(2, 2);
-          __builtin_amdgcn_sched_barrier(0);
-          FCVSR_RES_STEP(0);  FCVSR_RES_STEP(1);  FCVSR_RES_STEP(2);  FCVSR_RES_STEP(3);  FCVSR_RES_STEP(4);  FCVSR_RES_STEP(5);
-          FCVSR_RES_STEP(6);  FCVSR_RES_STEP(7);  FCVSR_RES_STEP(8);  FCVSR_RES_STEP(9);  FCVSR_RES_STEP(10); FCVSR_RES_STEP(11);
-          FCVSR_RES_STEP(12); FCVSR_RES_STEP(13); FCVSR_RES_STEP(14); FCVSR_RES_STEP(15); FCVSR_RES_STEP(16); FCVSR_RES_STEP(17);
-          FCVSR_RES_STEP(18); FCVSR_RES_STEP(19); FCVSR_RES_STEP(20); FCVSR_RES_STEP(21); FCVSR_RES_STEP(22); FCVSR_RES_STEP(23);
-          FCVSR_RES_STEP(24); FCVSR_RES_STEP(25); FCVSR_RES_STEP(26); FCVSR_RES_STEP(27); FCVSR_RES_STEP(28); FCVSR_RES_STEP(29);
-          FCVSR_RES_STEP(30); FCVSR_RES_STEP(31); FCVSR_RES_STEP(32); FCVSR_RES_STEP(33); FCVSR_RES_STEP(34); FCVSR_RES_STEP(35);
-#undef FCVSR_RES_STEP
-#undef FCVSR_RES_LOAD
-          __builtin_amdgcn_s_setprio(0);
-        }
-        asm volatile("s_waitcnt lgkmcnt(0)" ::: "memory");
-      }
-      __builtin_amdgcn_s_barrier();
-      if (act && ch == NCH - 1 && !(a.dbg & 8)) {
-        if (a.dbg & 32) __builtin_amdgcn_s_setprio(1);
-        const ResTile t = res_decode(tabP, a.n_groups, tile);
-        const int* T = tabP + t.gi * 32;
-        const int GH = T[kTH], GW = T[kTW];
-        gchar_t* dbase = tab_ptr(T, kTDstLo);
-        const int px = t.tx0 + r;
-        const float* bias_a = reinterpret_cast<const float*>(lds + kRBiasOff) + 16 * h;
-        const int cq4 = a.cout >> 2, sp = a.ps ? n0 / cq4 : 0, nch = a.ps ? n0 - sp * cq4 : n0;
-#pragma unroll
-        for (int j = 0; j < 2; ++j) {
-          uint2 pk[MF][4];
-#pragma unroll
-          for (int mf = 0; mf < MF; ++mf)
-#pragma unroll
-            for (int g = 0; g < 4; ++g) {
-              const float4 b4 = *reinterpret_cast<const float4*>(bias_a + mf * 32 + 4 * g);
-              float v[4] = {acc[mf][j][4 * g] + b4.x, acc[mf][j][4 * g + 1] + b4.y, acc[mf][j][4 * g + 2] + b4.z,
-                            acc[mf][j][4 * g + 3] + b4.w};
-#pragma unroll
-              for (int e = 0; e < 4; ++e)
-                if (NSU != 2) v[e] = NSU == 1 ? fmaxf(v[e], ns * v[e]) : fmaxf(v[e], 0.f) + ns * fminf(v[e], 0.f);
-              pk[mf][g] = cvt4<BF16>(make_float4(v[0], v[1], v[2], v[3]));
-            }
-          const int py = t.ty0 + 2 * wq + j;
-          const bool ok = (py < GH) && (px < GW) && !(a.dbg & 4);
-          const int pyc = ok ? py : 0, pxc = ok ? px : 0;
-          const int dyy = a.ps ? 2 * pyc + (sp >> 1) : pyc, dxx = a.ps ? 2 * pxc + (sp & 1) : pxc;
-          const unsigned dpix = (unsigned)(t.b * T[kTDstSb] + dyy * T[kTDstSy] + dxx * T[kTDstSx] + nch + 16 * h);
-          if (ok) {
-#pragma unroll
-            for (int mf = 0; mf < MF; ++mf)
-#pragma unroll
-              for (int q = 0; q < 2; ++q)
-                gstore(dbase + (size_t)(dpix + mf * 32 + 8 * q) * 2, make_uint4(pk[mf][2 * q].x, pk[mf][2 * q].y, pk[mf][2 * q + 1].x, pk[mf][2 * q + 1].y));
-          }
-        }
-      }
-      __builtin_amdgcn_s_barrier();
-    }
-  }
-  for (int i = 0; i < 2 - grp; ++i) __builtin_amdgcn_s_barrier();
-}
-
 bool conv3_res_supports(int cin, int cout) { return (cin == 64 && cout % 64 == 0) || (cin == 128 && cout % 32 == 0); }
 
 template <bool BF16, int MODE, int NCH, int NSU>
@@ -551,11 +387,7 @@
   static DevOnce attr;
   int dev = 0;
   hipError_t e = once_per_device(attr, [&] {
-    hipError_t e1 = hipFuncSetAttribute((const void*)conv3_res_kernel<BF16, MODE, NCH, NSU>, hipFuncAttributeMaxDynamicSharedMemorySize, (int)kRLds);
-    if constexpr (BF16 && MODE == 2)
-      if (e1 == hipSuccess)
-        e1 = hipFuncSetAttribute((const void*)conv3_res3_kernel<true, NCH, NSU, 3>, hipFuncAttributeMaxDynamicSharedMemorySize, (int)kRLds);
-    return e1;
+    return hipFuncSetAttribute((const void*)conv3_res_kernel<BF16, MODE, NCH, NSU>, hipFuncAttributeMaxDynamicSharedMemorySize, (int)kRLds);
   }, &dev);
   if (e != hipSuccess) return e;
   const int cus = device_cu_count(dev);
@@ -589,14 +421,7 @@
     put(kTR0Lo, r0.p); T[kTR0Sb] = (int)r0.sb; T[kTR0Sy] = (int)r0.sy; T[kTR0Sx] = (int)r0.sx;
     put(kTR1Lo, r1.p); T[kTR1Sb] = (int)r1.sb; T[kTR1Sy] = (int)r1.sy; T[kTR1Sx] = (int)r1.sx;
   }
-  bool v2 = false;
-  if constexpr (BF16 && MODE == 2) {
-    if (a.variant == 3) {
-      hipLaunchKernelGGL((conv3_res3_kernel<true, NCH, NSU, 3>), dim3(grid), dim3(768), kRLds, st, k);
-      v2 = true;
-    }
-  }
-  if (!v2) hipLaunchKernelGGL((conv3_res_kernel<BF16, MODE, NCH, NSU>), dim3(grid), dim3(512), kRLds, st, k);
+  hipLaunchKernelGGL((conv3_res_kernel<BF16, MODE, NCH, NSU>), dim3(grid), dim3(512), kRLds, st, k);
   return hipGetLastError();
 }
 
diff --git a/fcvsr_amd/csrc/mfma_util.h b/fcvsr_amd/csrc/mfma_util.h
--- a/fcvsr_amd/csrc/mfma_util.h
+++ b/fcvsr_amd/csrc/mfma_util.h
@@ -8,6 +8,7 @@
 typedef __attribute__((ext_vector_type(4))) __bf16 bf16x4_t;
 typedef __attribute__((ext_vector_type(4))) _Float16 f16x4_t;
 typedef __attribute__((ext_vector_type(16))) float f32x16_t;
+typedef __attribute__((ext_vector_type(4))) float f32x4_t;
 
 
 template <bool BF16>
@@ -27,6 +28,14 @@
     return __builtin_amdgcn_mfma_f32_32x32x16_bf16(__builtin_bit_cast(bf16x8_t, a), __builtin_bit_cast(bf16x8_t, b), c, 0, 0, 0);
   else
     return __builtin_amdgcn_mfma_f32_32x32x16_f16(__builtin_bit_cast(f16x8_t, a), __builtin_bit_cast(f16x8_t, b), c, 0, 0, 0);
+}
+
+template <bool BF16>
+__device__ __forceinline__ f32x4_t mfma16x16x32(uint4 a, uint4 b, f32x4_t c) {
+  if (BF16)
+    return __builtin_amdgcn_mfma_f32_16x16x32_bf16(__builtin_bit_cast(bf16x8_t, a), __builtin_bit_cast(bf16x8_t, b), c, 0, 0, 0);
+  else
+    return __builtin_amdgcn_mfma_f32_16x16x32_f16(__builtin_bit_cast(f16x8_t, a), __builtin_bit_cast(f16x8_t, b), c, 0, 0, 0);
 }
 
 template <bool BF16>
```
